# qiaozhijian/VCR-Net

Measured on AMD Instinct MI355X. Metric: point-cloud pairs/sec (N=1024, batch 16 per GPU), higher is better.
Workload: dtype f32; 1 GPU; BASELINE configs[1]: ModelNet40-like whole-to-whole registration, N=1024, batch=16 pairs per GPU, LPDNet(k=20)+Transformer+VcpTopK+SVD, iter=1, fp32; synthetic object clouds with the reference's transform recipe; LPD-pretrained emb_nn + seeded Transformer weights; num_points=1024, batch_per_gpu=16, global_batch=16, k=20, iters=1, parallelism=dp1 (pairs sharded per rank), entry_point=vcrnet_amd.module.vcrnetIter(net, src, tgt, iter) -> vcr_vcrnet_iter_f32

## Files before the change

vcr-net_amd/csrc/forward.hip:

```cpp
#include "common.h"

namespace {

enum Launch : int {
  STEM, KNN, TIE_REPLAY, EDGECONV, SN1_PQ, GATHERMAX, CONV3,
  ENCDEC_QKV, ENCDEC_SELF, WO_PAIR, FFN1_CROSS_Q, MERGED_ENC_FFN2,
  ENC_QKV = ENCDEC_QKV, ENC_SELF, ENC_WO, ENC_FFN1, ENC_FFN2, DEC_QKV, DEC_SELF, DEC_SELF_WO, DEC_CROSS_Q,
  DEC_CROSS_KV, CROSS_ATT, DEC_CROSS_WO, DEC_FFN1, DEC_FFN2, DEC_NORM, HEAD, HEAD2,
  END = HEAD2
};
static_assert(MERGED_ENC_FFN2 < DEC_CROSS_KV, "the merged first sublayers end in front of the positions both forms share");

struct Plan {
  struct Req { void** slot; size_t bytes; int birth, death; size_t off; };
  static constexpr int MAXR = 96;
  Req r[MAXR];
  int n = 0;
  bool overflow = false;
  bool flat = false;
  template <class T> void want(T*& field, size_t count, int birth, int death) {
    field = nullptr;
    if (count == 0) return;
    if (flat) { birth = 0; death = 1 << 30; }
    if (n >= MAXR) { overflow = true; return; }
    r[n++] = Req{reinterpret_cast<void**>(&field), (count * sizeof(T) + 255) & ~(size_t)255, birth, death, 0};
  }
  size_t solve(unsigned char* base) {
    int order[MAXR];
    for (int i = 0; i < n; ++i) order[i] = i;
    for (int i = 1; i < n; ++i) {
      const int x = order[i];
      int j = i - 1;
      while (j >= 0 && r[order[j]].bytes < r[x].bytes) { order[j + 1] = order[j]; --j; }
      order[j + 1] = x;
    }
    size_t total = 0;
    for (int oi = 0; oi < n; ++oi) {
      Req& q = r[order[oi]];
      size_t off = 0;
      for (bool moved = true; moved;) {
        moved = false;
        for (int pj = 0; pj < oi; ++pj) {
          const Req& p = r[order[pj]];
          if (p.death < q.birth || q.death < p.birth) continue;
          if (off < p.off + p.bytes && p.off < off + q.bytes) { off = p.off + p.bytes; moved = true; }
        }
      }
      q.off = off;
      if (off + q.bytes > total) total = off + q.bytes;
    }
    for (int i = 0; i < n; ++i) *r[i].slot = base + r[i].off;
    return total;
  }
};

struct Ws {
  float *xyz4, *feat64, *sq64, *pq1, *cat, *pq3, *emb;
  int32_t *idx1, *idx3, *ties;
  unsigned char* tie_work[2]; size_t tie_work_each;
  float* feat64t;
  float *feat_p, *xyz4_p, *cen64, *cen4, *sq_p, *c64_sq, *c64_rad, *c64_max, *c4_rad, *c4_max;
  int32_t *perm, *ord_ok;
  float *qkv, *att, *attx, *e1, *e2, *hid, *d1, *d2, *d3, *qc, *kvc, *embf, *side4, *csplit, *asplit;
  float* corr_ba;
  long asplit_floats;
  float *st_emb, *st_e1, *st_e2, *st_d1, *st_d2;
  float *rowstat, *keymass; uint8_t* keep;
  float* xsplit;
  float* xscore;
  int32_t* xorder;
  float *rstat, *cstat, *colsum, *rowsum, *score;
  float* rsplit;
  int32_t *sel_s, *sel_t, *amax, *pick;
  float *so_e, *to_e, *so_s, *to_s, *peak;
  float *eh1, *eh2, *eh3;
  float *cur_cf, *Ri, *ti, *Rb, *tb;
  size_t bytes;
};
inline size_t tgt_cache_floats(int B, int N, int E) { return (size_t)2 * B * N * 5 * E; }

inline int overlap_k1(int N, double o2) { return (int)((double)N * 0.84 * o2); }
inline int overlap_k2(int N, double o2) { return (int)((double)overlap_k1(N, o2) * 0.52 * o2); }

constexpr int KNN_ORDERED_MIN_N = 2048;
inline int merged_encdec(const vcr_vcrnet_weights* W) {
  return W->has_pointer == 1 && (W->linear_mode == 0 || W->split.encdec_qkv) && W->fold_encdec_qkv.w && W->fold_encdec_qkv.colsum &&
         W->fold_encdec_qkv.bias;
}

extern "C" int vcr_linear_shapes_(const vcr_linear_args* a, const vcr_linear_args* b, int* shape_a, int* shape_b);
extern "C" int vcr_knn_forms_(const vcr_knn_args* a, const vcr_knn_args* b, int* ordered, int* inline_a, int* inline_b);
extern "C" int vcr_sdpa_forms_(const vcr_sdpa_args* a, int* nsplit, int* persistent);
extern "C" long vcr_sdpa_split_floats_(size_t rows, int heads, int ldo, long nbatch, int nq, int cus);

Ws carve(void* base, const vcr_vcrnet_weights* W, int B, int N, int cus, int pass = 0) {
  const int k = W->k, E = W->E, F = W->F, heads = W->heads;
  const bool merged = merged_encdec(W) != 0;
  Plan pl;
  pl.flat = W->workspace_flat != 0;
  const size_t M = (size_t)2 * B * N;
  Ws w{};
  pl.want(w.xyz4, M * 4, STEM, END);   pl.want(w.feat64, M * 64, STEM, EDGECONV);   pl.want(w.sq64, M, STEM, TIE_REPLAY);
  pl.want(w.idx1, M * k, KNN, EDGECONV);   pl.want(w.idx3, M * k, KNN, GATHERMAX);   pl.want(w.ties, 2 * (1 + M), STEM, TIE_REPLAY);
  {
    const size_t slots = vcr_knn_tie_slot_bytes(2 * B, N);
    w.tie_work_each = (k > 20 && slots <= ((size_t)1 << 30)) ? slots : vcr_knn_tie_work_bytes(N);
    w.tie_work_each = (w.tie_work_each + 255) & ~(size_t)255;
  }
  pl.want(w.tie_work[0], w.tie_work_each ? 2 * w.tie_work_each : 0, KNN, TIE_REPLAY);
  pl.want(w.pq1, M * 256, STEM, SN1_PQ);   pl.want(w.cat, M * 512, EDGECONV, CONV3);   pl.want(w.pq3, M * 512, SN1_PQ, GATHERMAX);
  pl.want(w.emb, M * E, STEM, DEC_NORM);
  pl.want(w.qkv, M * 3 * E * (merged ? 2 : 1), merged ? ENCDEC_QKV : ENC_QKV, merged ? ENCDEC_SELF : DEC_SELF);
  pl.want(w.att, M * E * (merged ? 2 : 1), merged ? ENCDEC_SELF : ENC_SELF, merged ? WO_PAIR : DEC_SELF_WO);
  pl.want(w.e1, M * E, merged ? WO_PAIR : ENC_WO, merged ? MERGED_ENC_FFN2 : ENC_FFN2);
  pl.want(w.e2, M * E, merged ? MERGED_ENC_FFN2 : ENC_FFN2, DEC_CROSS_KV);
  pl.want(w.hid, M * F, merged ? FFN1_CROSS_Q : ENC_FFN1, DEC_FFN2);
  pl.want(w.d1, M * E, merged ? WO_PAIR : DEC_SELF_WO, DEC_CROSS_WO);
  pl.want(w.qc, M * E, merged ? FFN1_CROSS_Q : DEC_CROSS_Q, CROSS_ATT);   pl.want(w.kvc, M * 2 * E, DEC_CROSS_KV, CROSS_ATT);
  pl.want(w.attx, M * E, CROSS_ATT, DEC_CROSS_WO);
  pl.want(w.d2, M * E, DEC_CROSS_WO, END);
  pl.want(w.d3, M * E, DEC_FFN2, END);
  pl.want(w.embf, M * E, DEC_NORM, END);  pl.want(w.side4, M * 4, DEC_NORM, END);
  pl.want(w.csplit, VCR_PAIRSCORE_MAX_SPLIT * (M / 2) * 8, HEAD, END);
  pl.want(w.corr_ba, (size_t)B * N * 4, HEAD2, END);
  w.asplit_floats = vcr_sdpa_split_floats_(2 * M, heads, E, 2L * B, N, cus);
  pl.want(w.asplit, (size_t)w.asplit_floats, merged ? ENCDEC_SELF : ENC_SELF, CROSS_ATT);
  const size_t sn = M * (E / 64) * 2;
  pl.want(w.st_emb, sn, CONV3, DEC_QKV);
  pl.want(w.st_e1, sn, merged ? WO_PAIR : ENC_WO, merged ? FFN1_CROSS_Q : ENC_FFN1);
  pl.want(w.st_e2, sn, merged ? MERGED_ENC_FFN2 : ENC_FFN2, DEC_CROSS_KV);
  pl.want(w.st_d1, sn, merged ? WO_PAIR : DEC_SELF_WO, merged ? FFN1_CROSS_Q : DEC_CROSS_Q);
  pl.want(w.st_d2, sn, DEC_CROSS_WO, DEC_FFN1);
  const size_t K1 = (size_t)overlap_k1(N, W->overlap2), K2 = (size_t)overlap_k2(N, W->overlap2), B1 = (size_t)B;
  if (W->partial) {
    pl.want(w.rowstat, M * heads * 2, CROSS_ATT, CROSS_ATT); pl.want(w.keymass, M, CROSS_ATT, CROSS_ATT); pl.want(w.keep, M, CROSS_ATT, CROSS_ATT);
    pl.want(w.xsplit, VCR_SDPA_MAX_SPLIT * M * heads * 2, CROSS_ATT, CROSS_ATT);
    const size_t xs = M * heads * ((N + 31) & ~31);
    const int xmb = W->xscore_limit_mb;
    const size_t xlimit = xmb > 0 ? (size_t)xmb << 20 : xmb < 0 ? 0 : (size_t)4 << 30;
    pl.want(w.xscore, xs * 4 <= xlimit ? xs : 0, CROSS_ATT, CROSS_ATT);
    pl.want(w.xorder, M, CROSS_ATT, CROSS_ATT);
    pl.want(w.rstat, B1 * N * 2, HEAD, END); pl.want(w.cstat, B1 * N * 2, HEAD, END);
    pl.want(w.rsplit, VCR_PAIRSCORE_MAX_SPLIT * B1 * N * 2, HEAD, END);
    pl.want(w.rowsum, 2 * B1 * N, HEAD, END);
    pl.want(w.score, B1 * N * ((N + 31) & ~31), HEAD, END);
    pl.want(w.sel_s, 2 * B1 * K1, HEAD, END);
    pl.want(w.amax, B1 * K1, HEAD, END);     pl.want(w.pick, B1 * (K2 ? K2 : 1), HEAD, END);
    pl.want(w.so_e, 2 * B1 * K1 * E, HEAD, END);
    pl.want(w.so_s, 2 * B1 * K1 * 4, HEAD, END);
    pl.want(w.peak, B1 * K1 * 2, HEAD, END);
  }
  if (W->emb_kind == 1 && k != 20 && k != 40) {
    const size_t Mk = M * k;
    pl.want(w.eh1, Mk * 64, EDGECONV, GATHERMAX); pl.want(w.eh2, Mk * 64, EDGECONV, GATHERMAX);
    pl.want(w.eh3, Mk * 128, EDGECONV, GATHERMAX);
  }
  pl.want(w.cur_cf, (size_t)B * 3 * N, STEM, END);
  pl.want(w.Ri, (size_t)B * 9, STEM, END); pl.want(w.ti, (size_t)B * 3, STEM, END);
  pl.want(w.Rb, (size_t)B * 9, STEM, END); pl.want(w.tb, (size_t)B * 3, STEM, END);
  w.bytes = pl.solve(reinterpret_cast<unsigned char*>(base)) + 256;
  bool bad = pl.overflow;
  w.tie_work[1] = w.tie_work[0] ? w.tie_work[0] + w.tie_work_each : nullptr;
  if (W->partial) {
    w.colsum = w.rowsum + B1 * N;
    w.sel_t = w.sel_s + B1 * K1;
    w.to_e = w.so_e + B1 * K1 * E;
    w.to_s = w.so_s + B1 * K1 * 4;
  }
  if (pass != 0) {
    float* c = reinterpret_cast<float*>(static_cast<unsigned char*>(base) + w.bytes);
    w.emb = c;   c += M * E;
    w.d1 = c;    c += M * E;
    w.qc = c;    c += M * E;
    w.kvc = c;
  }
  w.feat64t = E >= 64 ? w.emb : nullptr;
  {
    const size_t T = (size_t)2 * B * ((N + 15) / 16);
    float* p = w.emb + M * 64;
    auto take = [&p](size_t n) { float* q = p; p += n; return q; };
    w.feat_p = take(M * 64);  w.xyz4_p = take(M * 4);  w.cen64 = take(T * 64);  w.cen4 = take(T * 4);  w.sq_p = take(M);
    w.perm = reinterpret_cast<int32_t*>(take(M));
    w.c64_sq = take(T);  w.c64_rad = take(T);  w.c64_max = take(T);  w.c4_rad = take(T);  w.c4_max = take(T);
    w.ord_ok = reinterpret_cast<int32_t*>(take(2 * B));
    if (pass != 0 && p > w.emb + B1 * N * E) bad = true;
  }
  if (bad) w.bytes = ~(size_t)0;
  return w;
}

__global__ __launch_bounds__(256) void zero_i32_kernel(int32_t* p, long n) {
  const long i = (long)blockIdx.x * 256 + threadIdx.x;
  if (i < n) p[i] = 0;
}

struct Runner {
  hipStream_t stream; vcr_trace* tr; int rc = 0;
  int shape_rows = 0;
  int plan_nbatch = 0;
  bool sdpa_split = false;
  float* pv_split = nullptr; long pv_split_floats = 0;
  int linear_variant = 0;
  int sdpa_variant = 0;
  vcr_knn_args deferred[2];
  int n_deferred = 0;

  void pin_shape(vcr_linear_args& a, vcr_linear_args* b = nullptr, int full_rows = 0) {
    const int fm = full_rows ? full_rows : shape_rows;
    if (!shape_rows || a.M >= fm || (a.variant & (16 | 1024))) return;
    vcr_linear_args fa = a, fb = b ? *b : a;
    fa.M = fm; fb.M = fm;
    int sa = 0, sb = 0;
    if (vcr_linear_shapes_(&fa, b ? &fb : nullptr, &sa, &sb) != VCR_OK) return;
    a.variant |= sa ? 16 : 1024;
    if (b) b->variant |= sb ? 16 : 1024;
  }
  bool ok(int r) { if (rc == 0 && r != 0) rc = r; return rc == 0; }
  template <class F> bool run(const char* name, F&& launch) {
    if (rc) return false;
    if (tr) {
      if (tr->count < VCR_TRACE_MAX) tr->names[tr->count] = name;
      if (tr->events && tr->count < tr->capacity) (void)hipEventRecord((hipEvent_t)tr->events[tr->count], stream);
      ++tr->count;
    }
    return ok(launch());
  }
  void finish() {
    if (tr && tr->events && tr->count < tr->capacity) (void)hipEventRecord((hipEvent_t)tr->events[tr->count], stream);
  }

  vcr_linear_args linear_args(const float* x, int ldx, const float* w, const float* b, float* y, int ldy, int M, int N, int K,
                              int relu, const float* res = nullptr, int ldr = 0, const float* ln_stats = nullptr,
                              const float* ln_colsum = nullptr, float* stats_out = nullptr) {
    vcr_linear_args a{x, ldx, w, b, res, ldr, y, ldy, M, N, K, relu};
    if (ln_stats) { a.ln_stats_in = ln_stats; a.ln_nseg = K / 64; a.ln_colsum = ln_colsum; a.ln_eps = 1e-6f; }
    a.stats_out = stats_out;
    a.variant = linear_variant;
    return a;
  }
  struct Lin { const char* name; vcr_linear_args a; const void* split; };
  bool linear(const Lin& l) {
    return run(l.name, [&] {
      vcr_linear_args a = l.a;
      if (!l.split) pin_shape(a);
      return l.split ? vcr_linear_bf16x3_f32(&a, l.split, stream) : vcr_linear_f32(&a, stream);
    });
  }
  bool linear(const char* nm, const float* x, int ldx, const float* w, const void* wsplit, const float* b, float* y,
              int ldy, int M, int N, int K, int relu, const float* res = nullptr, int ldr = 0,
              const float* ln_stats = nullptr, const float* ln_colsum = nullptr, float* stats_out = nullptr) {
    return linear({nm, linear_args(x, ldx, w, b, y, ldy, M, N, K, relu, res, ldr, ln_stats, ln_colsum, stats_out), wsplit});
  }
  bool linear2(const char* nm, vcr_linear_args a, vcr_linear_args b) {
    return run(nm, [&] {
      pin_shape(a, &b);
      return vcr_linear_pair_f32(&a, &b, stream);
    });
  }
  bool norm(const char* nm, const float* x, const vcr_norm_w& n, float* y, int M, int E,
            const float* res = nullptr, const float* xyz4 = nullptr, float* side4 = nullptr) {
    return run(nm, [&] {
      vcr_layernorm_args a{x, E, n.ln_a, n.ln_b, 1e-6f, res, E, y, E, M, E, xyz4, side4};
      return vcr_layernorm_f32(&a, stream);
    });
  }
  bool sdpa(const char* nm, const float* q, int ldq, const float* k, int ldk, const float* v, int ldv, float* out,
            int ldo, int nb, int heads, int nq, int nk, int shift, const uint8_t* keep = nullptr,
            float* rowstat = nullptr, float* score_out = nullptr, int ld_score = 0, int ngroups = 1, long in_group_stride = 0,
            long out_group_stride = 0, float* split_work = nullptr, long split_floats = 0) {
    return run(nm, [&] {
      vcr_sdpa_args a{q, ldq, k, ldk, v, ldv, out, ldo, nb, heads, nq, nk, 1.0f / sqrtf(128.f), shift, keep, rowstat,
                      score_out, ld_score};
      a.split_work = split_work ? split_work : out ? pv_split : nullptr;
      a.split_work_floats = split_work ? split_floats : out ? pv_split_floats : 0;
      if (ngroups > 1) {
        a.ngroups = ngroups; a.q_group_stride = a.k_group_stride = a.v_group_stride = in_group_stride;
        a.out_group_stride = out_group_stride;
      }
      a.variant = sdpa_variant;
      if (plan_nbatch > nb) a.plan_nbatch = plan_nbatch;
      return (sdpa_split && out && !rowstat && !score_out) ? vcr_sdpa_bf16x3_f32(&a, stream) : vcr_sdpa_f32(&a, stream);
    });
  }
  bool pairscore(const char* nm, const vcr_pairscore_args& a) {
    return run(nm, [&] { return vcr_pairscore_f32(&a, stream); });
  }
  bool rank(const char* nm, const float* values, int stride, int nb, int n, int K, int32_t* order, uint8_t* mask,
            int largest) {
    return run(nm, [&] {
      vcr_rankselect_args a{values, nb, n, K, order, mask, largest, stride};
      return vcr_rankselect_f32(&a, stream);
    });
  }
  bool gather(const char* nm, const float* in, int ld, int n_in, const int32_t* idx, int nb, int n_out, int C,
              float* out, const int32_t* via = nullptr, int n_via = 0) {
    return run(nm, [&] {
      vcr_gather_args a{in, ld, n_in, idx, nb, n_out, C, out, C, via, n_via};
      return vcr_gather_rows_f32(&a, stream);
    });
  }

  void knn(const char* nm, vcr_knn_args a) {
    a.tie_zeroed = 1;
    run(nm, [&] { return vcr_knn_f32(&a, stream); });
  }
  void knn_pair(const char* nm, vcr_knn_args a64, vcr_knn_args a3) {
    run(nm, [&] {
      a64.tie_zeroed = a3.tie_zeroed = 1;
      a64.tie_defer = a3.tie_defer = 1;
      n_deferred = 0;
      int inl64 = 0, inl3 = 0;
      (void)vcr_knn_forms_(&a64, &a3, nullptr, &inl64, &inl3);
      if (!inl64) deferred[n_deferred++] = a64;
      if (!inl3) deferred[n_deferred++] = a3;
      return vcr_knn_pair_f32(&a64, &a3, stream);
    });
  }
  void knn_ties() {
    if (n_deferred) run("knn:ties", [&] { return vcr_knn_ties_f32(&deferred[0], n_deferred == 2 ? &deferred[1] : nullptr, stream); });
    n_deferred = 0;
  }
  void copy_idx(const char* nm, int32_t* dst, const int32_t* src, size_t n) {
    run(nm, [&] { return vcr_copy_d2d(dst, src, n * sizeof(int32_t), stream); });
  }

  void cross_attention(const vcr_vcrnet_weights* W, const vcr_vcrnet_io* io, const Ws& w, int B, int N) {
    const int E = W->E, H = W->heads, nb = 2 * B, dk = E / H;
    const uint8_t* keep = nullptr;
    if (W->partial) {
      const int nkeep = (int)((double)N * W->overlap2);
      if (io->force_keys) {
        if (sdpa_split && W->F < 2 * E) { ok(VCR_EUNSUPPORTED); return; }
        copy_idx("select:dec.cross.keys.forced", w.xorder, io->force_keys, (size_t)nb * nkeep);
      } else if (w.xscore) {
        const int ldS = (N + 31) & ~31;
        sdpa("sdpa:dec.cross.stats", w.qc, E, w.kvc, 2 * E, nullptr, 0, nullptr, 0, nb, H, N, N, B, nullptr, w.rowstat,
             w.xscore, ldS, 1, 0, 0, w.xsplit, (long)VCR_SDPA_MAX_SPLIT * nb * H * N * 2);
        run("scoremass:dec.cross.keymass", [&] {
          vcr_keymass_args a{w.xscore, ldS, nb, H, N, N, w.rowstat, B, w.keymass};
          return vcr_keymass_f32(&a, stream);
        });
      } else {
        sdpa("sdpa:dec.cross.stats", w.qc, E, w.kvc, 2 * E, nullptr, 0, nullptr, 0, nb, H, N, N, B, nullptr, w.rowstat, nullptr, 0,
             1, 0, 0, w.xsplit, (long)VCR_SDPA_MAX_SPLIT * nb * H * N * 2);
        for (int h = 0; h < H; ++h) {
          vcr_pairscore_args a{};
          a.own = w.kvc + h * dk; a.ld_own = 2 * E; a.str = w.qc + h * dk; a.ld_str = E;
          a.nbatch = nb; a.n_own = N; a.n_str = N; a.E = dk; a.score = 1; a.scale = 1.0f / sqrtf((float)dk);
          a.str_batch_shift = B; a.op = 2; a.str_stat2 = w.rowstat + (size_t)h * N * 2;
          a.str_stat_batch_stride = (long)H * N * 2; a.mass = w.keymass; a.accumulate = h > 0;
          pairscore("pairscore:dec.cross.keymass", a);
        }
      }
      if (!io->force_keys) rank("select:dec.cross.keys", w.keymass, 1, nb, N, nkeep, w.xorder, w.keep, 1);
      if (io->out_keys) copy_idx("select:dec.cross.keys.out", io->out_keys, w.xorder, (size_t)nb * nkeep);
      vcr_sdpa_args xa{w.qc, E, w.kvc, 2 * E, w.kvc + E, 2 * E, w.attx, E, nb, H, N, nkeep, 1.0f / sqrtf(128.f), B};
      xa.key_index = w.xorder; xa.nk_src = N;
      if (!sdpa_split && vcr_sdpa_forms_(&xa, nullptr, nullptr) == VCR_OK) {
        run("sdpa:dec.cross", [&] { return vcr_sdpa_f32(&xa, stream); });
        return;
      }
      if (W->F >= 2 * E) {
        gather("select:gather.kv", w.kvc, 2 * E, N, w.xorder, nb, nkeep, 2 * E, w.hid);
        sdpa("sdpa:dec.cross", w.qc, E, w.hid, 2 * E, w.hid + E, 2 * E, w.attx, E, nb, H, N, nkeep, B);
        return;
      }
      keep = w.keep;
    }
    sdpa("sdpa:dec.cross", w.qc, E, w.kvc, 2 * E, w.kvc + E, 2 * E, w.attx, E, nb, H, N, N, B, keep);
  }

  void partial_head(const vcr_vcrnet_weights* W, const vcr_vcrnet_io* io, const Ws& w, int B, int N) {
    const int E = W->E, M1 = B * N;
    const int K1 = overlap_k1(N, W->overlap2), K2 = overlap_k2(N, W->overlap2);
    const float *se = w.embf, *te = w.embf + (size_t)M1 * E, *ss = w.side4, *ts = w.side4 + (size_t)M1 * 4;
    auto stats = [&](const char* nm, const float* own, const float* str, const float* os, const float* sd, int no,
                     int ns, float* stat2, int32_t* amax, float* score_out, int ld_score) {
      vcr_pairscore_args a{};
      a.own = own; a.ld_own = E; a.str = str; a.ld_str = E; a.own_side4 = os; a.str_side4 = sd;
      a.nbatch = B; a.n_own = no; a.n_str = ns; a.E = E; a.score = 0; a.scale = 1.f; a.op = 1;
      a.stat2 = stat2; a.argmax = amax; a.score_out = score_out; a.ld_score = ld_score;
      a.split_work = amax ? nullptr : w.rsplit;
      a.split_work_floats = amax ? 0 : (long)VCR_PAIRSCORE_MAX_SPLIT * B * N * 2;
      pairscore(nm, a);
    };
    const int ldS = (N + 31) & ~31;
    const bool forced_sets = io->force_sel_src && io->force_sel_tgt;
    if (!forced_sets) {
      stats("pairscore:head.scores", se, te, ss, ts, N, N, w.rstat, nullptr, w.score, ldS);
      run("scoremass:head", [&] {
        vcr_scoremass_args a{w.score, ldS, B, N, N, w.rstat, w.cstat, w.colsum, w.rowsum};
        return vcr_scoremass_f32(&a, stream);
      });
    }
    if (forced_sets) {
      copy_idx("select:head.tgt.forced", w.sel_t, io->force_sel_tgt, (size_t)B * K1);
      copy_idx("select:head.src.forced", w.sel_s, io->force_sel_src, (size_t)B * K1);
    } else {
      rank("select:head.src+tgt", w.rowsum, 1, 2 * B, N, K1, w.sel_s, nullptr, 1);
    }
    if (io->out_sel_tgt) copy_idx("select:head.tgt.out", io->out_sel_tgt, w.sel_t, (size_t)B * K1);
    if (io->out_sel_src) copy_idx("select:head.src.out", io->out_sel_src, w.sel_s, (size_t)B * K1);
    gather("select:gather.emb", se, E, N, w.sel_s, 2 * B, K1, E, w.so_e);
    gather("select:gather.xyz", ss, 4, N, w.sel_s, 2 * B, K1, 4, w.so_s);
    if (!(io->force_argmax && io->force_pairs))
      stats("pairscore:head.copair", w.so_e, w.to_e, w.so_s, w.to_s, K1, K1, w.peak, w.amax, nullptr, 0);
    if (io->force_argmax) copy_idx("select:head.argmax.forced", w.amax, io->force_argmax, (size_t)B * K1);
    if (io->force_pairs) copy_idx("select:head.pairs.forced", w.pick, io->force_pairs, (size_t)B * K2);
    else rank("select:head.pairs", w.peak + 1, 2, B, K1, K2, w.pick, nullptr, 0);
    if (io->out_argmax) copy_idx("select:head.argmax.out", io->out_argmax, w.amax, (size_t)B * K1);
    if (io->out_pairs) copy_idx("select:head.pairs.out", io->out_pairs, w.pick, (size_t)B * K2);
    gather("select:gather.srcK", w.so_s, 4, K1, w.pick, B, K2, 4, io->src4);
    gather("select:gather.corrK", w.to_s, 4, K1, w.pick, B, K2, 4, io->corr4, w.amax, K1);
    run("rigid_svd:ab", [&] {
      vcr_rigid_svd_args a{io->src4, 4, io->corr4, 4, B, K2, io->R_ab, io->t_ab, io->R_ba, io->t_ba, nullptr};
      return vcr_rigid_svd_f32(&a, stream);
    });
  }
};

int forward_impl(const vcr_vcrnet_weights* W, const vcr_vcrnet_io* io, void* workspace, size_t ws_bytes,
                 vcr_stream_t stream, vcr_trace* tr, bool last = true, int pass = 0) {
  if (!W || !io || !workspace || !io->src_cf || !io->tgt_cf || !io->corr4 || !io->src4 || !io->R_ab || !io->t_ab)
    return VCR_EINVAL;
  const int B = io->B, N = io->N, E = W->E, F = W->F, k = W->k;
  if (B <= 0 || N <= 0 || E != 512 || W->heads * 128 != E || k <= 0 || k + 1 > N) return VCR_EINVAL;
  if (k > 62 || N > 65535) return VCR_EUNSUPPORTED;
  if (W->emb_kind < 0 || W->emb_kind > 2) return VCR_EINVAL;
  if (W->emb_kind == 2 && !(W->c1_w && W->c1_b && W->c2_w && W->c2_b && W->pointnet.c3_w && W->pointnet.c3_b && W->pointnet.c4_w &&
                            W->pointnet.c4_b && W->pointnet.c5_w && W->pointnet.c5_b))
    return VCR_EINVAL;
  if (W->has_pointer == 1 && (F % 128)) return VCR_EINVAL;
  if (W->has_pointer == 1 &&
      !(W->fold_enc_qkv.w && W->fold_enc_ffn1.w && W->fold_dec_qkv.w && W->fold_dec_cross_q.w &&
        W->fold_dec_cross_kv.w && W->fold_dec_ffn1.w))
    return VCR_EINVAL;
  if (((uintptr_t)workspace) & 255) return VCR_EINVAL;
  if (W->head_mode < 0 || W->head_mode > 2 || W->linear_mode < 0 || W->linear_mode > 2) return VCR_EINVAL;
  for (int ms : {W->linear_mfma, W->linear_bk})
    if (ms != 0 && ms != 16 && ms != 32) return VCR_EINVAL;
  if ((W->linear_bm != 0 && W->linear_bm != 96 && W->linear_bm != 128) || (W->linear_bm == 96 && W->linear_mfma == 32)) return VCR_EINVAL;
  if (W->knn_waves != 0 && W->knn_waves != 1 && W->knn_waves != 8) return VCR_EINVAL;
  if (W->partial) {
    if (W->has_pointer != 1 || (W->cycle && W->head_mode == 0)) return VCR_EUNSUPPORTED;
    if (!(W->overlap2 > 0.0 && W->overlap2 <= 1.0) || (int)((double)N * W->overlap2) < 1) return VCR_EINVAL;
    if (W->head_mode == 0 && overlap_k2(N, W->overlap2) < 3) return VCR_EINVAL;
  }
  if (!W->partial && (io->force_keys || io->force_sel_src || io->force_sel_tgt || io->force_argmax || io->force_pairs))
    return VCR_EINVAL;
  if ((io->force_sel_src != nullptr) != (io->force_sel_tgt != nullptr)) return VCR_EINVAL;
  Ws w = carve(workspace, W, B, N, vcr_cu_count(), pass);
  if (ws_bytes < w.bytes) return VCR_EWORKSPACE;
  if (pass != 0 && ws_bytes < w.bytes + tgt_cache_floats(B, N, E) * sizeof(float)) return VCR_EINVAL;
  const int M1 = B * N, M2 = 2 * M1;
  const bool half = pass == 2;
  const int Bq = half ? B : 2 * B, Mq = half ? M1 : M2;
#define NM(site) (half ? site "@src" : site)
  Runner R{(hipStream_t)stream, tr};
  R.shape_rows = half ? M2 : 0;
  R.plan_nbatch = half ? 2 * B : 0;
  hipLaunchKernelGGL(zero_i32_kernel, dim3((unsigned)((M2 + 2 + 255) / 256)), dim3(256), 0, R.stream, w.ties, (long)(M2 + 2));
  R.ok(VCR_LAUNCH_RC());
#define SP(site) (W->linear_mode != 0 ? W->split.site : nullptr)
  R.sdpa_split = W->linear_mode == 2;
  R.sdpa_variant = W->sdpa_variant;
  R.pv_split = w.asplit; R.pv_split_floats = w.asplit_floats;
  R.linear_variant = (W->linear_mfma == 16 ? 16 : W->linear_mfma == 32 ? 1024 : 0) | (W->linear_bk == 16 ? 64 : W->linear_bk == 32 ? 8 : 0) |
                     (W->linear_bm == 96 ? 2048 : W->linear_bm == 128 ? 4096 : 0);

  const float* stats_for_ln = W->has_pointer == 1 ? w.st_emb : nullptr;
  if (W->emb_kind == 1) {
    for (int c = 0; c < (half ? 1 : 2); ++c) {
      R.run(c ? "pointwise:tgt" : "pointwise:src", [&] {
        return vcr_rows4_pq_f32(c ? io->tgt_cf : io->src_cf, w.xyz4 + (size_t)c * M1 * 4, B, N, W->dgcnn.c1_wpq, 32,
                                W->dgcnn.c1_bpq, 128, w.pq1 + (size_t)c * M1 * 128, 128, R.stream);
      });
    }
    {
      vcr_knn_args a3{(uint32_t)sizeof(vcr_knn_args), w.xyz4, 4, nullptr, Bq, N, 4, k, w.idx3, w.ties + 1 + M2, M2};
      a3.tie_work = w.tie_work[0]; a3.tie_work_bytes = w.tie_work_each;
      R.knn(NM("knn:xyz"), a3);
    }
    const int Mk = Mq * k;
    auto conv_max = [&](const char* nm, const float* x, int K, const float* wt, const float* bias, float* y, int Nout,
                        int col) {
      R.run(nm, [&] {
        vcr_linear_args a{x, K, wt, bias, nullptr, 0, y, Nout, Mk, Nout, K, 1};
        a.segmax_out = w.cat + col; a.ld_segmax = 512; a.seg_k = k;
        a.variant = R.linear_variant;
        R.pin_shape(a, nullptr, M2 * k);
        return vcr_linear_f32(&a, R.stream);
      });
    };
    if (k == 20 || k == 40) {
      R.run(NM("edgeconv:dg_chain"), [&] {
        vcr_edgechain_args a{w.pq1, 128, w.idx3, k, Mq, N, W->dgcnn.c2_w, W->dgcnn.c2_b, W->dgcnn.c3_w, W->dgcnn.c3_b,
                             W->dgcnn.c4_w, W->dgcnn.c4_b, w.cat, 512};
        return vcr_edgechain_f32(&a, R.stream);
      });
    } else {
      R.run(NM("gathermax:dg_c1"), [&] {
        vcr_edgerows_args a{w.pq1, 128, 64, w.idx3, k, Mq, N, w.eh1, 64, w.cat, 512, 512};
        return vcr_edgerows_f32(&a, R.stream);
      });
      conv_max(NM("linear:dg_c2"), w.eh1, 64, W->dgcnn.c2_w, W->dgcnn.c2_b, w.eh2, 64, 64);
      conv_max(NM("linear:dg_c3"), w.eh2, 64, W->dgcnn.c3_w, W->dgcnn.c3_b, w.eh3, 128, 128);
      conv_max(NM("linear:dg_c4"), w.eh3, 128, W->dgcnn.c4_w, W->dgcnn.c4_b, nullptr, 256, 256);
    }
    R.linear(NM("linear:conv3"), w.cat, 512, W->dgcnn.c5_w, nullptr, W->dgcnn.c5_b, w.emb, E, Mq, E, 512, 1, nullptr, 0, nullptr,
             nullptr, const_cast<float*>(stats_for_ln));
  } else if (W->emb_kind == 2) {
    R.run(NM("pointwise:src+tgt"), [&] {
      vcr_pointwise_args a{io->src_cf, B, N, W->c1_w, W->c1_b, W->c2_w, W->c2_b, w.xyz4, w.feat64, w.sq64, half ? nullptr : io->tgt_cf,
                           half ? 0 : B};
      return vcr_pointwise_f32(&a, R.stream);
    });
    R.linear(NM("linear:pn_c3"), w.feat64, 64, W->pointnet.c3_w, nullptr, W->pointnet.c3_b, w.pq1, 64, Mq, 64, 64, 1);
    R.linear(NM("linear:pn_c4"), w.pq1, 64, W->pointnet.c4_w, nullptr, W->pointnet.c4_b, w.cat, 128, Mq, 128, 64, 1);
    R.linear(NM("linear:pn_c5"), w.cat, 128, W->pointnet.c5_w, nullptr, W->pointnet.c5_b, w.emb, E, Mq, E, 128, 1, nullptr, 0, nullptr,
             nullptr, const_cast<float*>(stats_for_ln));
  } else {
  const bool pq_fused = W->linear_mode == 0;
  R.run(pq_fused ? NM("pointwise:src+tgt+dg1_pq") : NM("pointwise:src+tgt"), [&] {
    vcr_pointwise_args a{io->src_cf, B, N, W->c1_w, W->c1_b, W->c2_w, W->c2_b, w.xyz4, w.feat64, w.sq64, half ? nullptr : io->tgt_cf,
                         half ? 0 : B};
    if (pq_fused) { a.pq_w = W->dg1_wpq; a.pq_b = W->dg1_bpq; a.pq = w.pq1; a.ldpq = 256; }
    a.feat64t = w.feat64t;
    return vcr_pointwise_f32(&a, R.stream);
  });
  const int32_t* rank_perm = nullptr;
  {
    vcr_knn_args a64{(uint32_t)sizeof(vcr_knn_args), w.feat64, 64, w.sq64, Bq, N, 64, k, w.idx1, w.ties, M2, W->knn_waves};
    vcr_knn_args a3{(uint32_t)sizeof(vcr_knn_args), w.xyz4, 4, nullptr, Bq, N, 4, k, w.idx3, w.ties + 1 + M2, M2};
    a64.tie_work = w.tie_work[0]; a3.tie_work = w.tie_work[1];
    a64.tie_work_bytes = a3.tie_work_bytes = w.tie_work_each;
    a64.xt = w.feat64t;
    int pair_ordered = 0;
    if (R.rc == 0 && W->E >= 256 && N >= KNN_ORDERED_MIN_N && N <= 8192 && (k == 20 || k == 40) && W->knn_waves == 0 &&
        vcr_knn_forms_(&a64, &a3, &pair_ordered, nullptr, nullptr) == VCR_OK && pair_ordered) {
      R.run(NM("knn:rank"), [&] {
        vcr_knn_order_args o{w.xyz4, w.feat64t, 64, w.sq64, Bq, N, w.perm, w.xyz4_p, w.cen4, w.c4_rad, w.c4_max, w.feat_p, w.sq_p,
                             w.cen64, w.c64_sq, w.c64_rad, w.c64_max, w.ord_ok, nullptr, 0.f};
        return vcr_knn_order_f32(&o, R.stream);
      });
      a64.perm = a3.perm = w.perm;
      a64.ord_ok = w.ord_ok;
      rank_perm = w.perm;
      a64.xp = w.feat_p; a64.sqp = w.sq_p; a64.cen = w.cen64; a64.cen_sq = w.c64_sq; a64.cen_rad = w.c64_rad; a64.cen_sqmax = w.c64_max;
      a3.xp = w.xyz4_p; a3.cen = w.cen4; a3.cen_rad = w.c4_rad; a3.cen_sqmax = w.c4_max;
    }
    R.knn_pair(NM("knn:feat64+xyz"), a64, a3);
  }
  if (!pq_fused) R.linear(NM("linear:dg1_pq"), w.feat64, 64, W->dg1_wpq, SP(dg1_pq), W->dg1_bpq, w.pq1, 256, Mq, 256, 64, 0);
  R.knn_ties();
  R.run(NM("edgeconv:dg1_dg2"), [&] {
    vcr_edgeconv_args a{w.pq1, 256, w.idx1, k, Mq, N, W->dg2_w, W->dg2_b, w.cat, 512, w.cat + 128, 512};
    return W->linear_mode != 0 && (k == 20 || k == 40) ? vcr_edgeconv_bf16x3_f32(&a, R.stream) : vcr_edgeconv_f32(&a, R.stream);
  });
  R.linear(NM("linear:sn1_pq"), w.cat + 128, 512, W->sn1_wpq, SP(sn1_pq), W->sn1_bpq, w.pq3, 512, Mq, 512, 128, 0);
  R.run(NM("gathermax:sn1"), [&] {
    vcr_gathermax_args a{w.pq3, 512, 256, w.idx3, k, Mq, N, w.cat + 256, 512};
    a.order = rank_perm;
    return vcr_gathermax_f32(&a, R.stream);
  });
  R.linear(NM("linear:conv3"), w.cat, 512, W->c3_w, SP(c3), W->c3_b, w.emb, E, Mq, E, 512, 1, nullptr, 0, nullptr, nullptr,
           W->has_pointer == 1 ? w.st_emb : nullptr);

  }
  if (W->has_pointer != 1) { R.shape_rows = 0; R.plan_nbatch = 0; }

  const float* head_emb = w.embf;
  if (W->has_pointer == 1) {
    const int H = W->heads;
    const bool merged = merged_encdec(W) != 0;
    const float* att_dec = merged ? w.att + (size_t)M2 * E : w.att;
    using Lin = Runner::Lin;
    const Lin enc_wo{NM("linear:enc.wo"), R.linear_args(w.att, E, W->enc_self.wo, W->enc_self.bo, w.e1, E, Mq, E, E, 0, w.emb, E,
                                                         nullptr, nullptr, w.st_e1), SP(enc_wo)};
    const Lin dec_self_wo{NM("linear:dec.self.wo"), R.linear_args(att_dec, E, W->dec_self.wo, W->dec_self.bo, w.d1, E, Mq, E, E, 0,
                                                                  w.emb, E, nullptr, nullptr, w.st_d1), SP(dec_self_wo)};
    const Lin enc_ffn1{NM("linear:enc.ffn1"), R.linear_args(w.e1, E, W->fold_enc_ffn1.w, W->fold_enc_ffn1.bias, w.hid, F, Mq, F, E, 1,
                                                            nullptr, 0, w.st_e1, W->fold_enc_ffn1.colsum), SP(enc_ffn1)};
    const Lin dec_cross_q{NM("linear:dec.cross.q"), R.linear_args(w.d1, E, W->fold_dec_cross_q.w, W->fold_dec_cross_q.bias, w.qc, E, Mq,
                                                                  E, E, 0, nullptr, 0, w.st_d1, W->fold_dec_cross_q.colsum),
                          SP(dec_cross_q)};
    const Lin enc_ffn2{NM("linear:enc.ffn2"), R.linear_args(w.hid, F, W->enc_ffn.w2, W->enc_ffn.b2, w.e2, E, Mq, E, F, 0, w.e1, E,
                                                            nullptr, nullptr, w.st_e2), SP(enc_ffn2)};
    if (merged) {
      R.linear(NM("linear:encdec.qkv"), w.emb, E, W->fold_encdec_qkv.w, SP(encdec_qkv), W->fold_encdec_qkv.bias, w.qkv, 6 * E, Mq, 6 * E, E, 0,
               nullptr, 0, w.st_emb, W->fold_encdec_qkv.colsum);
      R.sdpa(NM("sdpa:encdec.self"), w.qkv, 6 * E, w.qkv + E, 6 * E, w.qkv + 2 * E, 6 * E, w.att, E, Bq, H, N, N, 0, nullptr, nullptr,
             nullptr, 0, 2, 3 * E, (long)M2 * E);
      if (W->linear_mode != 0) {
        R.linear(enc_wo); R.linear(dec_self_wo); R.linear(enc_ffn1); R.linear(dec_cross_q); R.linear(enc_ffn2);
      } else {
        R.linear2(NM("linear:enc.wo+dec.self.wo"), enc_wo.a, dec_self_wo.a);
        R.linear2(NM("linear:enc.ffn1+dec.cross.q"), enc_ffn1.a, dec_cross_q.a);
        R.linear(enc_ffn2);
      }
    } else {
      R.linear(NM("linear:enc.qkv"), w.emb, E, W->fold_enc_qkv.w, SP(enc_qkv), W->fold_enc_qkv.bias, w.qkv, 3 * E, Mq, 3 * E, E, 0,
               nullptr, 0, w.st_emb, W->fold_enc_qkv.colsum);
      R.sdpa(NM("sdpa:enc.self"), w.qkv, 3 * E, w.qkv + E, 3 * E, w.qkv + 2 * E, 3 * E, w.att, E, Bq, H, N, N, 0);
      R.linear(enc_wo); R.linear(enc_ffn1); R.linear(enc_ffn2);
      R.linear(NM("linear:dec.qkv"), w.emb, E, W->fold_dec_qkv.w, SP(dec_qkv), W->fold_dec_qkv.bias, w.qkv, 3 * E, Mq, 3 * E, E, 0,
               nullptr, 0, w.st_emb, W->fold_dec_qkv.colsum);
      R.sdpa(NM("sdpa:dec.self"), w.qkv, 3 * E, w.qkv + E, 3 * E, w.qkv + 2 * E, 3 * E, w.att, E, Bq, H, N, N, 0);
      R.linear(dec_self_wo); R.linear(dec_cross_q);
    }
    R.linear(NM("linear:dec.cross.kv"), w.e2, E, W->fold_dec_cross_kv.w, SP(dec_cross_kv), W->fold_dec_cross_kv.bias, w.kvc, 2 * E, Mq, 2 * E, E, 0,
             nullptr, 0, w.st_e2, W->fold_dec_cross_kv.colsum);
    R.shape_rows = 0; R.plan_nbatch = 0;
    R.cross_attention(W, io, w, B, N);
    R.linear("linear:dec.cross.wo", w.attx, E, W->dec_cross.wo, SP(dec_cross_wo), W->dec_cross.bo, w.d2, E, M2, E, E, 0, w.d1, E,
             nullptr, nullptr, w.st_d2);
    R.linear("linear:dec.ffn1", w.d2, E, W->fold_dec_ffn1.w, SP(dec_ffn1), W->fold_dec_ffn1.bias, w.hid, F, M2, F, E, 1, nullptr, 0,
             w.st_d2, W->fold_dec_ffn1.colsum);
    R.linear("linear:dec.ffn2", w.hid, F, W->dec_ffn.w2, SP(dec_ffn2), W->dec_ffn.b2, w.d3, E, M2, E, F, 0, w.d2, E);
    R.norm("layernorm:dec.norm+res", w.d3, W->dec_norm, w.embf, M2, E, w.emb, w.xyz4, w.side4);
  } else {
    R.run("layernorm:rowside", [&] {
      vcr_rowside_args a{w.emb, E, M2, E, W->has_pointer == 2 ? 2.f : 1.f, w.embf, E, w.xyz4, w.side4};
      return vcr_rowside_f32(&a, R.stream);
    });
  }

  const bool hard_pairs = W->partial && W->head_mode == 0;
  const float* side = w.side4;
  if (W->head_mode == 2) {
    if (!W->att_w0 || !W->att_w1) return VCR_EINVAL;
    R.linear("linear:head.att.src", w.embf, E, W->att_w0, nullptr, W->att_b0, w.d3, E, M1, E, E, 0);
    R.linear("linear:head.att.tgt", w.embf + (size_t)M1 * E, E, W->att_w1, nullptr, W->att_b1, w.d3 + (size_t)M1 * E, E,
             M1, E, E, 0);
    R.run("layernorm:rowside.att", [&] {
      vcr_rowside_args a{w.d3, E, M2, E, 1.f, nullptr, E, w.xyz4, w.side4};
      return vcr_rowside_f32(&a, R.stream);
    });
    head_emb = w.d3;
  }
  auto soft_head = [&](const char* nm, size_t q0, size_t k0, float* corr) {
    R.run(nm, [&] {
      vcr_softcorr_args a{head_emb + q0 * E, E, head_emb + k0 * E, E, side + q0 * 4, side + k0 * 4,
                          corr, B, N, N, E, W->head_mode == 1 ? 1 : 0, 1.0f / sqrtf((float)E), w.csplit,
                          (long)VCR_PAIRSCORE_MAX_SPLIT * B * N * 8};
      return vcr_softcorr_f32(&a, R.stream);
    });
  };
  if (hard_pairs) {
    R.partial_head(W, io, w, B, N);
  } else {
    soft_head("softcorr:head", 0, (size_t)M1, io->corr4);
    R.run("rigid_svd:ab", [&] {
      const int c = vcr_copy_d2d(io->src4, w.xyz4, (size_t)M1 * 4 * sizeof(float), R.stream);
      vcr_rigid_svd_args a{w.xyz4, 4, io->corr4, 4, B, N, io->R_ab, io->t_ab, io->R_ba, io->t_ba, nullptr};
      const int s = vcr_rigid_svd_f32(&a, R.stream);
      return c ? c : s;
    });
    if (W->cycle) {
      if (!io->R_ba || !io->t_ba) return VCR_EINVAL;
      if (W->head_mode == 2) {
        R.linear("linear:head.att.ba.src", w.embf, E, W->att_w1, nullptr, W->att_b1, w.d2, E, M1, E, E, 0);
        R.linear("linear:head.att.ba.tgt", w.embf + (size_t)M1 * E, E, W->att_w0, nullptr, W->att_b0, w.d2 + (size_t)M1 * E,
                 E, M1, E, E, 0);
        R.run("layernorm:rowside.att.ba", [&] {
          vcr_rowside_args a{w.d2, E, M2, E, 1.f, nullptr, E, w.xyz4, w.side4};
          return vcr_rowside_f32(&a, R.stream);
        });
        head_emb = w.d2;
      }
      soft_head("softcorr:head.ba", (size_t)M1, 0, w.corr_ba);
      R.run("rigid_svd:ba", [&] {
        vcr_rigid_svd_args a{w.xyz4 + (size_t)M1 * 4, 4, w.corr_ba, 4, B, N, io->R_ba, io->t_ba, nullptr, nullptr, nullptr};
        return vcr_rigid_svd_f32(&a, R.stream);
      });
    }
  }
  if (R.rc == 0 && io->emb_out) R.ok(vcr_copy_d2d(io->emb_out, w.embf, (size_t)M2 * E * sizeof(float), R.stream));
  if (last) R.finish();
#undef SP
#undef NM
  return R.rc;
}

__global__ __launch_bounds__(256) void pose_step_kernel(const float* __restrict__ Ri, const float* __restrict__ ti,
                                                        const float* in_cf, float* out_cf, int N, int compose,
                                                        float* Rf, float* tf, float* Rba, float* tba) {
  const int b = blockIdx.y;
  float r[9], t[3];
  for (int i = 0; i < 9; ++i) r[i] = Ri[b * 9 + i];
  for (int i = 0; i < 3; ++i) t[i] = ti[b * 3 + i];
  if (out_cf) {
    const int n = blockIdx.x * 256 + threadIdx.x;
    if (n < N) {
      const float* p = in_cf + (size_t)b * 3 * N + n;
      const float x = p[0], y = p[N], z = p[2 * (size_t)N];
      float* o = out_cf + (size_t)b * 3 * N + n;
      for (int c = 0; c < 3; ++c) o[(size_t)c * N] = fmaf(r[c * 3 + 2], z, fmaf(r[c * 3 + 1], y, r[c * 3] * x)) + t[c];
    }
  }
  if (compose == 2 && blockIdx.x == 0 && threadIdx.x == 0) {
    for (int i = 0; i < 3; ++i) {
      for (int j = 0; j < 3; ++j) Rba[b * 9 + i * 3 + j] = r[j * 3 + i];
      tba[b * 3 + i] = -fmaf(r[6 + i], t[2], fmaf(r[3 + i], t[1], r[i] * t[0]));
    }
  } else if (compose && blockIdx.x == 0 && threadIdx.x == 0) {
    float f[9], g[3], nf[9], ng[3];
    for (int i = 0; i < 9; ++i) f[i] = Rf[b * 9 + i];
    for (int i = 0; i < 3; ++i) g[i] = tf[b * 3 + i];
    for (int i = 0; i < 3; ++i) {
      for (int j = 0; j < 3; ++j) nf[i * 3 + j] = fmaf(r[i * 3 + 2], f[6 + j], fmaf(r[i * 3 + 1], f[3 + j], r[i * 3] * f[j]));
      ng[i] = fmaf(r[i * 3 + 2], g[2], fmaf(r[i * 3 + 1], g[1], r[i * 3] * g[0])) + t[i];
    }
    for (int i = 0; i < 9; ++i) Rf[b * 9 + i] = nf[i];
    for (int i = 0; i < 3; ++i) tf[b * 3 + i] = ng[i];
    for (int i = 0; i < 3; ++i) {
      for (int j = 0; j < 3; ++j) Rba[b * 9 + i * 3 + j] = nf[j * 3 + i];
      tba[b * 3 + i] = -fmaf(nf[6 + i], ng[2], fmaf(nf[3 + i], ng[1], nf[i] * ng[0]));
    }
  }
}

}

static int weights_take(const vcr_vcrnet_weights* user, vcr_vcrnet_weights* mine) {
  return vcr_take_args(user, mine, offsetof(vcr_vcrnet_weights, fold_encdec_qkv));
}

extern "C" size_t vcr_vcrnet_workspace_bytes(const vcr_vcrnet_weights* UW, int B, int N) {
  vcr_vcrnet_weights Wn;
  const vcr_vcrnet_weights* W = &Wn;
  if (weights_take(UW, &Wn) || B <= 0 || N <= 0) return 0;
  return carve(nullptr, W, B, N, vcr_cu_count()).bytes;
}

static bool iter_reuse_applies(const vcr_vcrnet_weights* W, int iters) { return iters > 1 && W->iter_reuse != 1; }
extern "C" size_t vcr_vcrnet_iter_workspace_bytes(const vcr_vcrnet_weights* UW, int B, int N, int iters) {
  vcr_vcrnet_weights Wn;
  const vcr_vcrnet_weights* W = &Wn;
  if (weights_take(UW, &Wn) || B <= 0 || N <= 0 || iters < 1) return 0;
  const size_t base = carve(nullptr, W, B, N, vcr_cu_count()).bytes;
  return base + (iter_reuse_applies(W, iters) ? tgt_cache_floats(B, N, W->E) * sizeof(float) : 0);
}

extern "C" int vcr_vcrnet_pairs(const vcr_vcrnet_weights* UW, int N) {
  vcr_vcrnet_weights Wn;
  const vcr_vcrnet_weights* W = &Wn;
  if (weights_take(UW, &Wn) || N <= 0) return 0;
  return (W->partial && W->head_mode == 0) ? overlap_k2(N, W->overlap2) : N;
}

extern "C" int vcr_vcrnet_forward_f32(const vcr_vcrnet_weights* UW, const vcr_vcrnet_io* io, void* ws, size_t bytes,
                                      vcr_stream_t stream) {
  vcr_vcrnet_weights Wn;
  if (weights_take(UW, &Wn)) return VCR_EINVAL;
  return forward_impl(&Wn, io, ws, bytes, stream, nullptr);
}

extern "C" int vcr_vcrnet_forward_traced_f32(const vcr_vcrnet_weights* UW, const vcr_vcrnet_io* io, void* ws,
                                             size_t bytes, vcr_stream_t stream, vcr_trace* tr) {
  vcr_vcrnet_weights Wn;
  if (weights_take(UW, &Wn)) return VCR_EINVAL;
  if (tr) tr->count = 0;
  return forward_impl(&Wn, io, ws, bytes, stream, tr);
}

extern "C" int vcr_vcrnet_iter_f32(const vcr_vcrnet_weights* UW, const vcr_vcrnet_io* io, int iters, void* ws,
                                   size_t bytes, vcr_stream_t stream, vcr_trace* tr) {
  vcr_vcrnet_weights Wn;
  const vcr_vcrnet_weights* W = &Wn;
  if (weights_take(UW, &Wn)) return VCR_EINVAL;
  if (!W || !io || iters < 1 || !io->R_ba || !io->t_ba) return VCR_EINVAL;
  if (tr) tr->count = 0;
  const int B = io->B, N = io->N;
  if (B <= 0 || N <= 0) return VCR_EINVAL;
  if (iters == 1) {
    const int rc = forward_impl(W, io, ws, bytes, stream, tr, !W->cycle);
    if (rc || !W->cycle) return rc;
    Runner R{(hipStream_t)stream, tr};
    R.run("pose:inverse", [&] {
      hipLaunchKernelGGL(pose_step_kernel, dim3(1, B), dim3(64), 0, R.stream, io->R_ab, io->t_ab, nullptr, nullptr, N, 2, nullptr,
                         nullptr, io->R_ba, io->t_ba);
      return VCR_LAUNCH_RC();
    });
    R.finish();
    return R.rc;
  }
  const Ws w = carve(ws, W, B, N, vcr_cu_count());
  if (bytes < w.bytes) return VCR_EWORKSPACE;
  const bool reuse = iter_reuse_applies(W, iters) && bytes >= w.bytes + tgt_cache_floats(B, N, W->E) * sizeof(float);
  const size_t nkeys = W->partial ? (size_t)2 * B * (int)((double)N * W->overlap2) : 0;
  const size_t nsel = W->partial ? (size_t)B * overlap_k1(N, W->overlap2) : 0;
  const size_t npair = W->partial ? (size_t)B * overlap_k2(N, W->overlap2) : 0;
  for (int it = 0; it < iters; ++it) {
    vcr_vcrnet_io step = *io;
    if (it > 0) { step.src_cf = w.cur_cf; step.R_ab = w.Ri; step.t_ab = w.ti; step.R_ba = w.Rb; step.t_ba = w.tb; }
    if (it + 1 < iters) step.emb_out = nullptr;
    auto at = [it](auto* p, size_t n) { return p ? p + (size_t)it * n : p; };
    step.force_keys = at(io->force_keys, nkeys);       step.out_keys = at(io->out_keys, nkeys);
    step.force_sel_src = at(io->force_sel_src, nsel);  step.out_sel_src = at(io->out_sel_src, nsel);
    step.force_sel_tgt = at(io->force_sel_tgt, nsel);  step.out_sel_tgt = at(io->out_sel_tgt, nsel);
    step.force_argmax = at(io->force_argmax, nsel);    step.out_argmax = at(io->out_argmax, nsel);
    step.force_pairs = at(io->force_pairs, npair);     step.out_pairs = at(io->out_pairs, npair);
    const bool last = it + 1 == iters;
    const int rc = forward_impl(W, &step, ws, bytes, stream, tr, false, reuse ? (it == 0 ? 1 : 2) : 0);
    if (rc) return rc;
    if (last && it == 0) break;
    Runner R{(hipStream_t)stream, tr};
    R.run("pose:step", [&] {
      hipLaunchKernelGGL(pose_step_kernel, dim3((N + 255) / 256, B), dim3(256), 0, R.stream, step.R_ab, step.t_ab, step.src_cf,
                         last ? nullptr : w.cur_cf, N, it > 0 ? 1 : 0, io->R_ab, io->t_ab, io->R_ba, io->t_ba);
      return VCR_LAUNCH_RC();
    });
    if (R.rc) return R.rc;
    if (last) R.finish();
  }
  return VCR_OK;
}

extern "C" int vcr_pose_step_f32(const vcr_pose_step_args* a, vcr_stream_t stream) {
  if (!a || !a->R_i || !a->t_i || a->B <= 0 || a->compose < 0 || a->compose > 2) return VCR_EINVAL;
  if ((a->out_cf != nullptr) != (a->in_cf != nullptr) || (a->out_cf && a->N <= 0)) return VCR_EINVAL;
  if (a->compose && (!a->R_ba || !a->t_ba)) return VCR_EINVAL;
  if (a->compose == 1 && (!a->R_f || !a->t_f)) return VCR_EINVAL;
  if (!a->compose && !a->out_cf) return VCR_OK;
  const int gx = a->out_cf ? (a->N + 255) / 256 : 1;
  hipLaunchKernelGGL(pose_step_kernel, dim3(gx, a->B), dim3(a->out_cf ? 256 : 64), 0, (hipStream_t)stream, a->R_i, a->t_i,
                     a->in_cf, a->out_cf, a->N, a->compose, a->R_f, a->t_f, a->R_ba, a->t_ba);
  return VCR_LAUNCH_RC();
}

extern "C" const char* vcr_strerror(int code) {
  switch (code) {
    case VCR_OK: return "ok";
    case VCR_EINVAL: return "invalid argument (shape, pitch, alignment or null pointer)";
    case VCR_EWORKSPACE: return "workspace too small";
    case VCR_EUNSUPPORTED: return "unsupported configuration";
    default: return code > 0 ? hipGetErrorString((hipError_t)code) : "unknown error";
  }
}

extern "C" int vcr_abi_version(void) { return VCR_ABI_VERSION; }

extern "C" int vcr_event_create(void** ev) {
  if (!ev) return VCR_EINVAL;
  hipEvent_t e;
  const hipError_t rc = hipEventCreate(&e);
  *ev = rc == hipSuccess ? (void*)e : nullptr;
  return (int)rc;
}
extern "C" int vcr_event_destroy(void* ev) { return ev ? (int)hipEventDestroy((hipEvent_t)ev) : VCR_EINVAL; }
extern "C" int vcr_event_record(void* ev, vcr_stream_t stream) {
  return ev ? (int)hipEventRecord((hipEvent_t)ev, (hipStream_t)stream) : VCR_EINVAL;
}
extern "C" int vcr_event_elapsed_ms(void* start, void* stop, float* ms) {
  if (!start || !stop || !ms) return VCR_EINVAL;
  return (int)hipEventElapsedTime(ms, (hipEvent_t)start, (hipEvent_t)stop);
}
```

vcr-net_amd/csrc/pairscore.hip:

```cpp
#include "common.h"

namespace {

constexpr float LOG2E = 1.4426950408889634f;

__device__ __forceinline__ bool argmax_before(float v, int i, float bv, int bi) {
  const bool vn = v != v, bn = bv != bv;
  return vn ? (!bn || i < bi) : (!bn && (v > bv || (v == bv && i < bi)));
}

template <int OP, int OT>
__global__ __launch_bounds__(128 * OT * 2, (OT == 1 ? 2 : 1)) void pairscore_kernel(vcr_pairscore_args p, int nsplit) {
  extern __shared__ __attribute__((aligned(16))) unsigned char smem[];
  constexpr int NW = 4 * OT;
  constexpr int NO = 32 * OT;
  const int QP = p.E + 4;
  float* Os = reinterpret_cast<float*>(smem);
  float* mg = Os + NO * QP;
  const int t = threadIdx.x, lane = t & 63, w = t >> 6;
  const int half = lane >> 5, l31 = lane & 31;
  int bx, b;
  xcd_chunk2(bx, b);
  const int sp = bx % nsplit;
  bx /= nsplit;
  const int o0 = bx * NO;
  const int sb = (b + p.str_batch_shift) % p.nbatch;
  const int chunks = p.E / 64;

  {
    const int per_row = p.E / 4;
    for (int i = t; i < NO * per_row; i += 64 * NW) {
      const int row = i / per_row, c4 = (i % per_row) * 4;
      const int orow = min(o0 + row, p.n_own - 1);
      st4(&Os[row * QP + c4], ld4(p.own + ((size_t)b * p.n_own + orow) * p.ld_own + c4));
    }
  }
  size_t own_row[OT];
  float own_norm[OT];
#pragma unroll
  for (int ot = 0; ot < OT; ++ot) {
    own_row[ot] = (size_t)b * p.n_own + min(o0 + 32 * ot + l31, p.n_own - 1);
    own_norm[ot] = p.score == 1 ? 0.f : p.own_side4[own_row[ot] * 4 + 3];
  }
  __syncthreads();

  const int ntiles_all = (p.n_str + 31) / 32;
  const int per_split = (ntiles_all + nsplit - 1) / nsplit, t0 = sp * per_split;
  const int ntiles = max(0, min(ntiles_all, t0 + per_split) - t0);
  const int my_tiles = max(0, (ntiles - w + NW - 1) / NW);
  const int nflat = my_tiles * chunks;
  const float* sbase = p.str + (size_t)sb * p.n_str * p.ld_str;
  const float* sside = p.str_side4 ? p.str_side4 + (size_t)sb * p.n_str * 4 : nullptr;
  const float* sstat = (OP == 2) ? p.str_stat2 + (size_t)sb * p.str_stat_batch_stride : nullptr;

  f32x4 bufA[8], bufB[8];
  auto load_chunk = [&](int flat, f32x4* dst) {
    const int tile = t0 + w + NW * (flat / chunks), c = flat % chunks;
    const int row = min(tile * 32 + l31, p.n_str - 1);
    const float* kp = sbase + (size_t)row * p.ld_str + 64 * c + 4 * half;
#pragma unroll
    for (int g = 0; g < 8; ++g) dst[g] = ld4(kp + 8 * g);
  };

  float m[OT], l[OT], ox[OT], oy[OT], oz[OT];
  float best[OT]; int bidx[OT];
  float mass[OT];
  f32x16 s[OT];
#pragma unroll
  for (int ot = 0; ot < OT; ++ot) {
    m[ot] = VCR_NEG_INF; l[ot] = ox[ot] = oy[ot] = oz[ot] = 0.f; best[ot] = VCR_NEG_INF; bidx[ot] = 0x7fffffff;
    mass[ot] = 0.f; s[ot] = f32x16{0};
  }
  f32x16 tot[OT];
  auto compute = [&](int flat, const f32x4* kf) {
    const int tile = t0 + w + NW * (flat / chunks), c = flat % chunks;
#pragma unroll
    for (int ot = 0; ot < OT; ++ot) s[ot] = f32x16{0};
#pragma unroll
    for (int g = 0; g < 8; ++g) {
#pragma unroll
      for (int ot = 0; ot < OT; ++ot) {
        const f32x4 qv = ld4(&Os[(32 * ot + l31) * QP + 64 * c + 8 * g + 4 * half]);
#pragma unroll
        for (int e = 0; e < 4; ++e) s[ot] = mfma32(kf[g][e], qv[e], s[ot]);
      }
    }
#pragma unroll
    for (int ot = 0; ot < OT; ++ot) {
      if (c == 0) tot[ot] = s[ot];
      else tot[ot] += s[ot];
    }
    if (c != chunks - 1) return;
    float rn = 0.f;
    if (p.score == 2) rn = sside[(size_t)min(tile * 32 + l31, p.n_str - 1) * 4 + 3];
    f32x4 side[16];
    if (OP == 0 || p.score == 0) {
#pragma unroll
      for (int r = 0; r < 16; ++r) side[r] = ld4(sside + (size_t)min(tile * 32 + acc_row(r, half), p.n_str - 1) * 4);
    }
#pragma unroll
    for (int ot = 0; ot < OT; ++ot) {
      f32x16& sc16 = tot[ot];
      if (p.score == 0) sc16 = mfma32(half == 0 ? 1.f : 0.f, half == 0 ? -0.5f * own_norm[ot] : 0.f, sc16);
      else if (p.score == 2) sc16 = mfma32(half == 0 ? -0.5f * rn : 0.f, half == 0 ? 1.f : 0.f, sc16);
      float mt = VCR_NEG_INF;
#pragma unroll
      for (int r = 0; r < 16; ++r) {
        const int j = tile * 32 + acc_row(r, half);
        float sc;
        if (p.score == 0) sc = 2.f * sc16[r] - side[r][3];
        else if (p.score == 2) sc = 2.f * sc16[r] - own_norm[ot];
        else sc = sc16[r] * p.scale;
        sc16[r] = j < p.n_str ? sc : VCR_NEG_INF;
        mt = fmaxf(mt, sc16[r]);
      }
      if (OP == 1 && p.score_out && o0 + 32 * ot + l31 < p.n_own) {
        float* srow = p.score_out + (own_row[ot] * (size_t)p.ld_score) + tile * 32 + 4 * half;
#pragma unroll
        for (int r4 = 0; r4 < 4; ++r4)
          st4(srow + 8 * r4, f32x4{sc16[4 * r4], sc16[4 * r4 + 1], sc16[4 * r4 + 2], sc16[4 * r4 + 3]});
      }
      if (OP == 2) {
#pragma unroll
        for (int r = 0; r < 16; ++r) {
          const int jc = min(tile * 32 + acc_row(r, half), p.n_str - 1);
          const float ms = sstat[(size_t)jc * 2], ls = sstat[(size_t)jc * 2 + 1];
          mass[ot] += __builtin_amdgcn_exp2f((sc16[r] - ms) * LOG2E) / ls;
        }
        continue;
      }
      if (OP == 1) {
#pragma unroll
        for (int r = 0; r < 16; ++r) {
          const int j = tile * 32 + acc_row(r, half);
          if (sc16[r] > best[ot] || (sc16[r] != sc16[r] && best[ot] == best[ot])) { best[ot] = sc16[r]; bidx[ot] = j; }
        }
      }
      mt = fmaxf(mt, xhalf(mt));
      const float m_new = fmaxf(m[ot], mt);
      const float alpha = __builtin_amdgcn_exp2f((m[ot] - m_new) * LOG2E);
      float ls = 0.f, ax = 0.f, ay = 0.f, az = 0.f;
#pragma unroll
      for (int r = 0; r < 16; ++r) {
        const float pr = __builtin_amdgcn_exp2f((sc16[r] - m_new) * LOG2E);
        ls += pr;
        if (OP == 0) { ax = fmaf(pr, side[r][0], ax); ay = fmaf(pr, side[r][1], ay); az = fmaf(pr, side[r][2], az); }
      }
      l[ot] = l[ot] * alpha + ls;
      if (OP == 0) { ox[ot] = ox[ot] * alpha + ax; oy[ot] = oy[ot] * alpha + ay; oz[ot] = oz[ot] * alpha + az; }
      m[ot] = m_new;
    }
  };

  if (nflat > 0) {
    load_chunk(0, bufA);
    int f = 0;
    for (; f + 2 < nflat; f += 2) {
      load_chunk(f + 1, bufB);
      __builtin_amdgcn_sched_barrier(0);
      compute(f, bufA);
      load_chunk(f + 2, bufA);
      __builtin_amdgcn_sched_barrier(0);
      compute(f + 1, bufB);
    }
    load_chunk(f + 1, bufB);
    __builtin_amdgcn_sched_barrier(0);
    compute(f, bufA);
    compute(f + 1, bufB);
  }

#pragma unroll
  for (int ot = 0; ot < OT; ++ot) {
    float* g = mg + (w * NO + 32 * ot + l31) * 5;
    if (OP == 2) {
      mass[ot] += xhalf(mass[ot]);
      if (half == 0) g[0] = mass[ot];
    } else {
      l[ot] += xhalf(l[ot]);
      if (OP == 0) { ox[ot] += xhalf(ox[ot]); oy[ot] += xhalf(oy[ot]); oz[ot] += xhalf(oz[ot]); }
      if (OP == 1) {
        const float ob = xhalf(best[ot]);
        const int oi = __shfl_xor(bidx[ot], 32, 64);
        if (argmax_before(ob, oi, best[ot], bidx[ot])) { best[ot] = ob; bidx[ot] = oi; }
      }
      if (half == 0) {
        g[0] = m[ot]; g[1] = l[ot];
        if (OP == 0) { g[2] = ox[ot]; g[3] = oy[ot]; g[4] = oz[ot]; }
        else { g[2] = best[ot]; g[3] = __int_as_float(bidx[ot]); }
      }
    }
  }
  __syncthreads();
  if (t < NO && o0 + t < p.n_own) {
    const size_t orow = (size_t)b * p.n_own + o0 + t;
    if (OP == 2) {
      float acc = 0.f;
#pragma unroll
      for (int i = 0; i < NW; ++i) acc += mg[(i * NO + t) * 5];
      p.mass[orow] = p.accumulate ? p.mass[orow] + acc : acc;
      return;
    }
    float M = VCR_NEG_INF;
#pragma unroll
    for (int i = 0; i < NW; ++i) M = fmaxf(M, mg[(i * NO + t) * 5]);
    float L = 0.f, X = 0.f, Y = 0.f, Z = 0.f, Bv = VCR_NEG_INF;
    int Bi = 0x7fffffff;
#pragma unroll
    for (int i = 0; i < NW; ++i) {
      const float* g = mg + (i * NO + t) * 5;
      const float a = g[0] == VCR_NEG_INF ? 0.f : __builtin_amdgcn_exp2f((g[0] - M) * LOG2E);
      L = fmaf(g[1], a, L);
      if (OP == 0) { X = fmaf(g[2], a, X); Y = fmaf(g[3], a, Y); Z = fmaf(g[4], a, Z); }
      else {
        const int gi = __float_as_int(g[3]);
        if (argmax_before(g[2], gi, Bv, Bi)) { Bv = g[2]; Bi = gi; }
      }
    }
    if (OP == 0) {
      if (nsplit > 1) {
        float* pw = p.split_work + ((size_t)sp * p.nbatch * p.n_own + orow) * 8;
        st4(pw, f32x4{M, L, X, Y});
        pw[4] = Z;
      } else {
        st4(p.corr4 + orow * 4, f32x4{X / L, Y / L, Z / L, 0.f});
      }
    } else {
      float* st = nsplit > 1 ? p.split_work + (size_t)sp * p.nbatch * p.n_own * 2 : p.stat2;
      st[orow * 2] = M; st[orow * 2 + 1] = L;
      if (p.argmax) p.argmax[orow] = Bi < p.n_str ? Bi : 0;
    }
  }
}

__global__ __launch_bounds__(256) void corrmerge_kernel(const float* part, int nsplit, long rows, float* corr4) {
  const long r = (long)blockIdx.x * 256 + threadIdx.x;
  if (r >= rows) return;
  float M = VCR_NEG_INF;
  for (int s = 0; s < nsplit; ++s) M = fmaxf(M, part[((size_t)s * rows + r) * 8]);
  float L = 0.f, X = 0.f, Y = 0.f, Z = 0.f;
  for (int s = 0; s < nsplit; ++s) {
    const float* g = part + ((size_t)s * rows + r) * 8;
    const float a = g[0] == VCR_NEG_INF ? 0.f : __builtin_amdgcn_exp2f((g[0] - M) * LOG2E);
    L = fmaf(g[1], a, L); X = fmaf(g[2], a, X); Y = fmaf(g[3], a, Y); Z = fmaf(g[4], a, Z);
  }
  st4(corr4 + r * 4, f32x4{X / L, Y / L, Z / L, 0.f});
}

__global__ __launch_bounds__(256) void statmerge_kernel(const float* part, int nsplit, long rows, float* stat2) {
  const long r = (long)blockIdx.x * 256 + threadIdx.x;
  if (r >= rows) return;
  float M = VCR_NEG_INF;
  for (int s = 0; s < nsplit; ++s) M = fmaxf(M, part[((size_t)s * rows + r) * 2]);
  float L = 0.f;
  for (int s = 0; s < nsplit; ++s) {
    const float* g = part + ((size_t)s * rows + r) * 2;
    L = fmaf(g[1], g[0] == VCR_NEG_INF ? 0.f : __builtin_amdgcn_exp2f((g[0] - M) * LOG2E), L);
  }
  stat2[r * 2] = M; stat2[r * 2 + 1] = L;
}

__global__ __launch_bounds__(256) void score_colpass_kernel(vcr_scoremass_args p) {
  __shared__ float mg[4][64][3];
  const int b = blockIdx.y, lane = threadIdx.x & 63, w = threadIdx.x >> 6;
  const int j = blockIdx.x * 64 + lane, jc = min(j, p.n_cols - 1);
  const float* S = p.score + (size_t)b * p.n_rows * p.ld + jc;
  const float* rs = p.row_stat2 + (size_t)b * p.n_rows * 2;
  const int per = (p.n_rows + 3) / 4, i0 = w * per, i1 = min(p.n_rows, i0 + per);
  float cm = VCR_NEG_INF, cl = 0.f, mass = 0.f;
  auto step = [&](float v, float mi, float li) {
    mass += __builtin_amdgcn_exp2f((v - mi) * LOG2E) / li;
    if (v > cm) { cl *= __builtin_amdgcn_exp2f((cm - v) * LOG2E); cm = v; }
    cl += __builtin_amdgcn_exp2f((v - cm) * LOG2E);
  };
  int i = i0;
  for (; i + 8 <= i1; i += 8) {
    float v[8], m8[8], l8[8];
#pragma unroll
    for (int u = 0; u < 8; ++u) { v[u] = S[(size_t)(i + u) * p.ld]; m8[u] = rs[2 * (i + u)]; l8[u] = rs[2 * (i + u) + 1]; }
#pragma unroll
    for (int u = 0; u < 8; ++u) step(v[u], m8[u], l8[u]);
  }
  for (; i < i1; ++i) step(S[(size_t)i * p.ld], rs[2 * i], rs[2 * i + 1]);
  mg[w][lane][0] = cm; mg[w][lane][1] = cl; mg[w][lane][2] = mass;
  __syncthreads();
  if (w == 0 && j < p.n_cols) {
    float M = VCR_NEG_INF, L = 0.f, A = 0.f;
    for (int q = 0; q < 4; ++q) M = fmaxf(M, mg[q][lane][0]);
    for (int q = 0; q < 4; ++q) {
      L = fmaf(mg[q][lane][1], __builtin_amdgcn_exp2f((mg[q][lane][0] - M) * LOG2E), L);
      A += mg[q][lane][2];
    }
    const size_t o = (size_t)b * p.n_cols + j;
    p.col_stat2[o * 2] = M; p.col_stat2[o * 2 + 1] = L;
    p.col_mass[o] = A;
  }
}

__global__ __launch_bounds__(256) void score_rowpass_kernel(vcr_scoremass_args p) {
  const int b = blockIdx.y, lane = threadIdx.x & 63;
  const int i = blockIdx.x * 4 + (threadIdx.x >> 6);
  if (i >= p.n_rows) return;
  const float* S = p.score + ((size_t)b * p.n_rows + i) * p.ld;
  const float* cs = p.col_stat2 + (size_t)b * p.n_cols * 2;
  float acc = 0.f;
#pragma unroll 4
  for (int j = lane; j < p.n_cols; j += 64)
    acc += __builtin_amdgcn_exp2f((S[j] - cs[2 * j]) * LOG2E) / cs[2 * j + 1];
#pragma unroll
  for (int off = 32; off > 0; off >>= 1) acc += __shfl_xor(acc, off, 64);
  if (lane == 0) p.row_mass[(size_t)b * p.n_rows + i] = acc;
}

enum class PsMerge { none, corr, stat };
struct PairscorePlan {
  int op, ot;
  int nsplit;
  dim3 grid, block; int lds;
  PsMerge merge; long rows; dim3 merge_grid;
};

int pairscore_plan(const vcr_pairscore_args* a, PairscorePlan* p) {
  if (!a || !a->own || !a->str) return VCR_EINVAL;
  if (a->nbatch <= 0 || a->n_own <= 0 || a->n_str <= 0 || a->E <= 0 || (a->E % 128) || a->E > 1024) return VCR_EINVAL;
  if ((a->ld_own & 3) || (a->ld_str & 3) || a->ld_own < a->E || a->ld_str < a->E) return VCR_EINVAL;
  if (a->score < 0 || a->score > 2 || a->op < 0 || a->op > 2) return VCR_EINVAL;
  if (a->score != 1 && (!a->own_side4 || !a->str_side4)) return VCR_EINVAL;
  if (a->op == 0 && (!a->corr4 || !a->str_side4)) return VCR_EINVAL;
  if (a->op == 1 && !a->stat2) return VCR_EINVAL;
  if (a->op == 2 && (!a->mass || !a->str_stat2)) return VCR_EINVAL;
  if (a->score_out && (a->op != 1 || (a->ld_score & 3) || a->ld_score < ((a->n_str + 31) & ~31))) return VCR_EINVAL;
  const int lds2 = (64 * (a->E + 4) + 8 * 64 * 5) * 4, lds1 = (32 * (a->E + 4) + 4 * 32 * 5) * 4;
  const int ot = (lds2 <= 160 * 1024 && a->E >= 256 && !(a->variant & 1)) ? 2 : 1;
  const int lds = ot == 2 ? lds2 : lds1;
  if (lds > 160 * 1024) return VCR_EUNSUPPORTED;
  const int owner_blocks = (a->n_own + 32 * ot - 1) / (32 * ot);
  int nsplit = 1;
  if ((a->op == 0 || (a->op == 1 && !a->argmax)) && a->split_work && !(a->variant & 4)) {
    const long blocks = (long)owner_blocks * a->nbatch, slots = (long)vcr_cu_count() * (ot == 2 ? 1 : 2);
    const int ntiles = (a->n_str + 31) / 32;
    double best = (double)((blocks + slots - 1) / slots);
    const double base = best;
    for (int sp = 2; sp <= VCR_PAIRSCORE_MAX_SPLIT; ++sp) {
      if (ntiles / sp < 4 * ot || (sp - 1) * ((ntiles + sp - 1) / sp) >= ntiles) break;
      const double c = (double)((blocks * sp + slots - 1) / slots) / sp;
      const long need = (long)sp * a->nbatch * a->n_own * (a->op == 0 ? 8 : 2);
      if (need > a->split_work_floats) break;
      if (c < 0.8 * base && c < best - 1e-9) { best = c; nsplit = sp; }
    }
  }
  const long rows = (long)a->nbatch * a->n_own;
  *p = PairscorePlan{a->op, ot, nsplit, dim3(owner_blocks * nsplit, a->nbatch), dim3(256 * ot), lds,
                     nsplit == 1 ? PsMerge::none : a->op == 0 ? PsMerge::corr : PsMerge::stat, rows, dim3((unsigned)((rows + 255) / 256))};
  return VCR_OK;
}

}

extern "C" int vcr_pairscore_f32(const vcr_pairscore_args* a, vcr_stream_t stream) {
  vcr_stream_scope bound(stream);
  PairscorePlan p;
  int rc = pairscore_plan(a, &p);
  if (rc) return rc;
  hipStream_t s = (hipStream_t)stream;
#define VCR_PS(OP, OT) rc = vcr_launch<pairscore_kernel<OP, OT>>(p.grid, p.block, p.lds, s, *a, p.nsplit)
  if (p.ot == 2) { if (p.op == 0) VCR_PS(0, 2); else if (p.op == 1) VCR_PS(1, 2); else VCR_PS(2, 2); }
  else           { if (p.op == 0) VCR_PS(0, 1); else if (p.op == 1) VCR_PS(1, 1); else VCR_PS(2, 1); }
#undef VCR_PS
  if (rc || p.merge == PsMerge::none) return rc;
  if (p.merge == PsMerge::corr) hipLaunchKernelGGL(corrmerge_kernel, p.merge_grid, dim3(256), 0, s, a->split_work, p.nsplit, p.rows, a->corr4);
  else hipLaunchKernelGGL(statmerge_kernel, p.merge_grid, dim3(256), 0, s, a->split_work, p.nsplit, p.rows, a->stat2);
  return VCR_LAUNCH_RC();
}

extern "C" int vcr_scoremass_f32(const vcr_scoremass_args* a, vcr_stream_t stream) {
  if (!a || !a->score || !a->row_stat2 || !a->col_stat2 || !a->col_mass || !a->row_mass) return VCR_EINVAL;
  if (a->nbatch <= 0 || a->n_rows <= 0 || a->n_cols <= 0 || a->ld < a->n_cols) return VCR_EINVAL;
  hipStream_t s = (hipStream_t)stream;
  hipLaunchKernelGGL(score_colpass_kernel, dim3((a->n_cols + 63) / 64, a->nbatch), dim3(256), 0, s, *a);
  hipLaunchKernelGGL(score_rowpass_kernel, dim3((a->n_rows + 3) / 4, a->nbatch), dim3(256), 0, s, *a);
  return VCR_LAUNCH_RC();
}

extern "C" int vcr_softcorr_f32(const vcr_softcorr_args* a, vcr_stream_t stream) {
  if (!a || !a->qside4 || !a->kside4 || !a->corr4) return VCR_EINVAL;
  if (a->mode != 0 && a->mode != 1) return VCR_EINVAL;
  vcr_pairscore_args p{};
  p.own = a->q; p.ld_own = a->ldq; p.str = a->k; p.ld_str = a->ldk;
  p.own_side4 = a->qside4; p.str_side4 = a->kside4;
  p.nbatch = a->nbatch; p.n_own = a->nq; p.n_str = a->nk; p.E = a->E;
  p.score = a->mode; p.scale = a->scale; p.str_batch_shift = 0; p.op = 0; p.corr4 = a->corr4;
  p.split_work = a->split_work; p.split_work_floats = a->split_work_floats;
  return vcr_pairscore_f32(&p, stream);
}
```

vcr-net_amd/csrc/pointwise.hip:

```cpp
#include "common.h"

namespace {

constexpr int PTS = 64;

__global__ __launch_bounds__(256) void pointwise12_kernel(vcr_pointwise_args a) {
  __shared__ float w2t[64][64];
  __shared__ float h1s[PTS][65];
  __shared__ float w1s[64][4];
  __shared__ float b2s[64];
  const int t = threadIdx.x;
  {
    f32x4 wv[4];
#pragma unroll
    for (int u = 0; u < 4; ++u) wv[u] = ld4(a.w2 + 4 * (t + 256 * u));
#pragma unroll
    for (int u = 0; u < 4; ++u) {
      const int i = 4 * (t + 256 * u), c = i >> 6, k = i & 63;
#pragma unroll
      for (int e = 0; e < 4; ++e) w2t[k + e][c] = wv[u][e];
    }
  }
  if (t < 64) {
    w1s[t][0] = a.w1[t * 3 + 0]; w1s[t][1] = a.w1[t * 3 + 1]; w1s[t][2] = a.w1[t * 3 + 2];
    w1s[t][3] = a.b1[t]; b2s[t] = a.b2[t];
  }
  const int b = blockIdx.y;
  const int p = t >> 2, g = t & 3;
  const int n = blockIdx.x * PTS + p;
  const bool live = n < a.N;
  const int nc = live ? n : a.N - 1;
  const float* xb = b < a.B ? a.x_cf + (size_t)b * 3 * a.N : a.x_cf2 + (size_t)(b - a.B) * 3 * a.N;
  const float x = xb[nc], y = xb[a.N + nc], z = xb[2 * a.N + nc];
  __syncthreads();
#pragma unroll
  for (int j = 0; j < 16; ++j) {
    const int c = g * 16 + j;
    const float v = fmaf(w1s[c][2], z, fmaf(w1s[c][1], y, fmaf(w1s[c][0], x, w1s[c][3])));
    h1s[p][c] = fmaxf(v, 0.f);
  }
  __syncthreads();
  float acc[16];
#pragma unroll
  for (int j = 0; j < 16; ++j) acc[j] = b2s[g * 16 + j];
  for (int k = 0; k < 64; ++k) {
    const float h = h1s[p][k];
#pragma unroll
    for (int q = 0; q < 4; ++q) {
      const f32x4 w = ld4(&w2t[k][g * 16 + q * 4]);
      acc[q * 4 + 0] = fmaf(w[0], h, acc[q * 4 + 0]);
      acc[q * 4 + 1] = fmaf(w[1], h, acc[q * 4 + 1]);
      acc[q * 4 + 2] = fmaf(w[2], h, acc[q * 4 + 2]);
      acc[q * 4 + 3] = fmaf(w[3], h, acc[q * 4 + 3]);
    }
  }
  float ss = 0.f;
#pragma unroll
  for (int j = 0; j < 16; ++j) {
    acc[j] = fmaxf(acc[j], 0.f);
    ss = ss + acc[j] * acc[j];
  }
  const int base = (threadIdx.x & 63) & ~3;
  {
    const float b0 = __shfl(ss, base, 64), b1 = __shfl(ss, base + 1, 64);
    const float b2 = __shfl(ss, base + 2, 64), b3 = __shfl(ss, base + 3, 64);
    ss = ((b0 + b1) + b2) + b3;
  }
  const bool tail = live && n >= (a.N & ~31);
  if (__builtin_amdgcn_ballot_w64(tail) != 0) {
    float a4[4] = {0.f, 0.f, 0.f, 0.f};
#pragma unroll
    for (int sgrp = 0; sgrp < 4; ++sgrp) {
      if (g == sgrp) {
#pragma unroll
        for (int j = 0; j < 16; ++j) a4[j & 3] = a4[j & 3] + acc[j] * acc[j];
      }
#pragma unroll
      for (int l = 0; l < 4; ++l) a4[l] = __shfl(a4[l], base + sgrp, 64);
    }
    if (tail) ss = ((a4[0] + a4[1]) + a4[2]) + a4[3];
  }
  if (live) {
    const size_t row = (size_t)b * a.N + n;
    float* o = a.feat64 + row * 64 + g * 16;
#pragma unroll
    for (int q = 0; q < 4; ++q) st4(o + q * 4, f32x4{acc[q * 4], acc[q * 4 + 1], acc[q * 4 + 2], acc[q * 4 + 3]});
    if (a.feat64t) {
      float* ot = a.feat64t + row * 64 + g * 16;
#pragma unroll
      for (int q = 0; q < 4; ++q) st4(ot + q * 4, f32x4{acc[q], acc[4 + q], acc[8 + q], acc[12 + q]});
    }
    if (g == 0) {
      a.sq64[row] = ss;
      st4(a.xyz4 + row * 4, f32x4{x, y, z, (x * x + y * y) + z * z});
    }
  }
}

constexpr int TP = 68;
constexpr int PQW = 8;
__global__ __launch_bounds__(64 * PQW, 1) void pointwise12_pq_kernel(vcr_pointwise_args a, int tiles_per_cloud, int total_tiles) {
  extern __shared__ __attribute__((aligned(16))) float pw_smem[];
  float* wfrag = pw_smem;
  float* w1s = wfrag + 16 * 4 * 64 * 4;
  float* pqb = w1s + 64 * 4;
  float* tiles = pqb + 256;
  const int t = threadIdx.x, lane = t & 63, wave = t >> 6;
  const int q4 = lane >> 4, l15 = lane & 15;
  f32x4 w2c[4][4];
#pragma unroll
  for (int j = 0; j < 4; ++j)
#pragma unroll
    for (int g = 0; g < 4; ++g) w2c[j][g] = ld4(a.w2 + (16 * j + l15) * 64 + 16 * g + 4 * q4);
  float b2r[4];
#pragma unroll
  for (int j = 0; j < 4; ++j) b2r[j] = a.b2[16 * j + l15];
  f32x4 wq[8];
#pragma unroll
  for (int it = 0; it < 8; ++it) wq[it] = ld4(a.pq_w + 4 * (t + 64 * PQW * it));
  if (t >= 256) pqb[t - 256] = a.pq_b[t - 256];
  if (t < 64) {
    w1s[t * 4 + 0] = a.w1[t * 3 + 0]; w1s[t * 4 + 1] = a.w1[t * 3 + 1]; w1s[t * 4 + 2] = a.w1[t * 3 + 2];
    w1s[t * 4 + 3] = a.b1[t];
  }
  float w2r[4][16];
#pragma unroll
  for (int j = 0; j < 4; ++j)
#pragma unroll
    for (int g = 0; g < 4; ++g) {
      int r0 = __float_as_int(w2c[j][g][0]), r1 = __float_as_int(w2c[j][g][1]);
      int r2 = __float_as_int(w2c[j][g][2]), r3 = __float_as_int(w2c[j][g][3]);
      auto s01 = __builtin_amdgcn_permlane16_swap(r0, r1, false, false); r0 = s01[0]; r1 = s01[1];
      auto s23 = __builtin_amdgcn_permlane16_swap(r2, r3, false, false); r2 = s23[0]; r3 = s23[1];
      auto s02 = __builtin_amdgcn_permlane32_swap(r0, r2, false, false); r0 = s02[0]; r2 = s02[1];
      auto s13 = __builtin_amdgcn_permlane32_swap(r1, r3, false, false); r1 = s13[0]; r3 = s13[1];
      w2r[j][4 * g] = __int_as_float(r0); w2r[j][4 * g + 1] = __int_as_float(r1);
      w2r[j][4 * g + 2] = __int_as_float(r2); w2r[j][4 * g + 3] = __int_as_float(r3);
    }
#pragma unroll
  for (int it = 0; it < 8; ++it) {
    const int c = t + 64 * PQW * it, n = c >> 4, st = c & 15, j = n >> 4;
#pragma unroll
    for (int e = 0; e < 4; ++e) wfrag[(((j * 4 + (st >> 2)) * 64) + e * 16 + (n & 15)) * 4 + (st & 3)] = wq[it][e];
  }
  __syncthreads();
  float* T = tiles + wave * 16 * TP;
  const int p = lane >> 2, g = lane & 3;
  for (int tile = (int)blockIdx.x * PQW + wave; tile < total_tiles; tile += (int)gridDim.x * PQW) {
    const int b = tile / tiles_per_cloud, n0 = (tile - b * tiles_per_cloud) * 16;
    const float* xb = b < a.B ? a.x_cf + (size_t)b * 3 * a.N : a.x_cf2 + (size_t)(b - a.B) * 3 * a.N;
    float h[16];
    {
      const int nc = min(n0 + l15, a.N - 1);
      const float x = xb[nc], y = xb[a.N + nc], z = xb[2 * a.N + nc];
#pragma unroll
      for (int st = 0; st < 16; ++st) {
        const f32x4 w = ld4(&w1s[(4 * st + q4) * 4]);
        h[st] = fmaxf(fmaf(w[2], z, fmaf(w[1], y, fmaf(w[0], x, w[3]))), 0.f);
      }
    }
    f32x4 acc[4];
#pragma unroll
    for (int j = 0; j < 4; ++j) acc[j] = f32x4{b2r[j], b2r[j], b2r[j], b2r[j]};
#pragma unroll
    for (int st = 0; st < 16; ++st)
#pragma unroll
      for (int j = 0; j < 4; ++j) acc[j] = mfma16(h[st], w2r[j][st], acc[j]);
#pragma unroll
    for (int j = 0; j < 4; ++j)
#pragma unroll
      for (int r = 0; r < 4; ++r) T[(4 * q4 + r) * TP + 16 * j + l15] = fmaxf(acc[j][r], 0.f);
    __builtin_amdgcn_s_waitcnt(0xc07f);
    __builtin_amdgcn_wave_barrier();
    auto feature_epilogue = [&]() {
      const int n = n0 + p;
      const bool live = n < a.N;
      const int nc = live ? n : a.N - 1;
      const float x = xb[nc], y = xb[a.N + nc], z = xb[2 * a.N + nc];
      float f[16];
#pragma unroll
      for (int q = 0; q < 4; ++q) {
        const f32x4 v = ld4(&T[p * TP + 16 * g + 4 * q]);
        f[4 * q] = v[0]; f[4 * q + 1] = v[1]; f[4 * q + 2] = v[2]; f[4 * q + 3] = v[3];
      }
      float ss = 0.f;
#pragma unroll
      for (int j = 0; j < 16; ++j) ss = ss + f[j] * f[j];
      const int base = lane & ~3;
      {
        const float s0 = __shfl(ss, base, 64), s1 = __shfl(ss, base + 1, 64);
        const float s2 = __shfl(ss, base + 2, 64), s3 = __shfl(ss, base + 3, 64);
        ss = ((s0 + s1) + s2) + s3;
      }
      const bool tail = live && n >= (a.N & ~31);
      if (__builtin_amdgcn_ballot_w64(tail) != 0) {
        float a4[4] = {0.f, 0.f, 0.f, 0.f};
#pragma unroll
        for (int sgrp = 0; sgrp < 4; ++sgrp) {
          if (g == sgrp) {
#pragma unroll
            for (int j = 0; j < 16; ++j) a4[j & 3] = a4[j & 3] + f[j] * f[j];
          }
#pragma unroll
          for (int l = 0; l < 4; ++l) a4[l] = __shfl(a4[l], base + sgrp, 64);
        }
        if (tail) ss = ((a4[0] + a4[1]) + a4[2]) + a4[3];
      }
      if (live) {
        const size_t row = (size_t)b * a.N + n;
        float* o = a.feat64 + row * 64 + g * 16;
#pragma unroll
        for (int q = 0; q < 4; ++q) st4(o + q * 4, f32x4{f[q * 4], f[q * 4 + 1], f[q * 4 + 2], f[q * 4 + 3]});
        if (a.feat64t) {
          float* ot = a.feat64t + row * 64 + g * 16;
#pragma unroll
          for (int q = 0; q < 4; ++q) st4(ot + q * 4, f32x4{f[q], f[4 + q], f[8 + q], f[12 + q]});
        }
        if (g == 0) {
          a.sq64[row] = ss;
          st4(a.xyz4 + row * 4, f32x4{x, y, z, (x * x + y * y) + z * z});
        }
      }
    };
    auto pq_product = [&]() {
    float af[16];
#pragma unroll
    for (int st = 0; st < 16; ++st) af[st] = T[l15 * TP + 4 * st + q4];
#pragma unroll 1
    for (int jg = 0; jg < 4; ++jg) {
      f32x4 pa[4];
#pragma unroll
      for (int jj = 0; jj < 4; ++jj) {
        const float bq = pqb[16 * (4 * jg + jj) + l15];
        pa[jj] = f32x4{bq, bq, bq, bq};
      }
#pragma unroll
      for (int sq = 0; sq < 4; ++sq)
#pragma unroll
        for (int jj = 0; jj < 4; ++jj) {
          const f32x4 wf = ld4(&wfrag[(((4 * jg + jj) * 4 + sq) * 64 + lane) * 4]);
#pragma unroll
          for (int e = 0; e < 4; ++e) pa[jj] = mfma16(af[4 * sq + e], wf[e], pa[jj]);
        }
#pragma unroll
      for (int jj = 0; jj < 4; ++jj)
#pragma unroll
        for (int r = 0; r < 4; ++r) {
          const int n = n0 + 4 * q4 + r;
          if (n < a.N) a.pq[((size_t)b * a.N + n) * a.ldpq + 16 * (4 * jg + jj) + l15] = pa[jj][r];
        }
    }
    };
    if (wave < PQW / 2) {
      feature_epilogue();
      pq_product();
    } else {
      pq_product();
      feature_epilogue();
    }
    __builtin_amdgcn_s_waitcnt(0xc07f);
    __builtin_amdgcn_wave_barrier();
  }
}

__global__ __launch_bounds__(256) void rows4_kernel(const float* x_cf, float* xyz4, int B, int N) {
  const long i = (long)blockIdx.x * 256 + threadIdx.x;
  if (i >= (long)B * N) return;
  const int b = (int)(i / N), n = (int)(i % N);
  const float* xb = x_cf + (size_t)b * 3 * N;
  const float x = xb[n], y = xb[N + n], z = xb[2 * N + n];
  st4(xyz4 + i * 4, f32x4{x, y, z, (x * x + y * y) + z * z});
}

__global__ __launch_bounds__(256) void rows4_pq_kernel(const float* x_cf, float* xyz4, int B, int N, const float* wpq,
                                                       int ldw, const float* bpq, int C, float* pq, int ldpq) {
  const int per = C / 4, cg = threadIdx.x % per;
  const long i = (long)blockIdx.x * (256 / per) + threadIdx.x / per;
  if (i >= (long)B * N) return;
  const int b = (int)(i / N), n = (int)(i % N);
  const float* xb = x_cf + (size_t)b * 3 * N;
  const float x = xb[n], y = xb[N + n], z = xb[2 * N + n];
  if (cg == 0) st4(xyz4 + i * 4, f32x4{x, y, z, (x * x + y * y) + z * z});
  f32x4 o;
#pragma unroll
  for (int e = 0; e < 4; ++e) {
    const float* wr = wpq + (size_t)(4 * cg + e) * ldw;
    o[e] = fmaf(wr[2], z, fmaf(wr[1], y, wr[0] * x)) + bpq[4 * cg + e];
  }
  st4(pq + i * ldpq + 4 * cg, o);
}

}

extern "C" int vcr_rows4_pq_f32(const float* x_cf, float* xyz4, int B, int N, const float* wpq, int ldw, const float* bpq,
                                int C, float* pq, int ldpq, vcr_stream_t stream) {
  if (!x_cf || !xyz4 || !wpq || !bpq || !pq || B <= 0 || N <= 0) return VCR_EINVAL;
  if (C <= 0 || (C % 4) || 256 % (C / 4) || ldw < 3 || ldpq < C || (ldpq & 3) || ((uintptr_t)pq & 15)) return VCR_EINVAL;
  const int pts = 256 / (C / 4);
  hipLaunchKernelGGL(rows4_pq_kernel, dim3((unsigned)(((long)B * N + pts - 1) / pts)), dim3(256), 0, (hipStream_t)stream,
                     x_cf, xyz4, B, N, wpq, ldw, bpq, C, pq, ldpq);
  return VCR_LAUNCH_RC();
}

extern "C" int vcr_rows4_f32(const float* x_cf, float* xyz4, int B, int N, vcr_stream_t stream) {
  if (!x_cf || !xyz4 || B <= 0 || N <= 0) return VCR_EINVAL;
  hipLaunchKernelGGL(rows4_kernel, dim3((unsigned)(((long)B * N + 255) / 256)), dim3(256), 0, (hipStream_t)stream, x_cf,
                     xyz4, B, N);
  return VCR_LAUNCH_RC();
}

extern "C" int vcr_pointwise_f32(const vcr_pointwise_args* a, vcr_stream_t stream) {
  vcr_stream_scope bound(stream);
  if (!a || !a->x_cf || !a->w1 || !a->b1 || !a->w2 || !a->b2 || !a->xyz4 || !a->feat64 || !a->sq64) return VCR_EINVAL;
  if (((uintptr_t)a->w2 | (uintptr_t)a->pq_w) & 15) return VCR_EINVAL;
  if (a->B <= 0 || a->N <= 0 || a->B2 < 0 || (a->B2 > 0 && !a->x_cf2)) return VCR_EINVAL;
  if (a->pq) {
    if (!a->pq_w || !a->pq_b || a->ldpq < 256 || (a->ldpq & 3)) return VCR_EINVAL;
    const int tpc = (a->N + 15) / 16, total = tpc * (a->B + a->B2);
    const int cus = vcr_cu_count(), blocks = (total + PQW - 1) / PQW < cus ? (total + PQW - 1) / PQW : cus;
    const size_t lds = (size_t)(16 * 4 * 64 * 4 + 64 * 4 + 256 + PQW * 16 * TP) * sizeof(float);
    VCR_DYN_LDS(pointwise12_pq_kernel, lds);
    hipLaunchKernelGGL(pointwise12_pq_kernel, dim3(blocks), dim3(64 * PQW), lds, (hipStream_t)stream, *a, tpc, total);
    return VCR_LAUNCH_RC();
  }
  dim3 grid((a->N + PTS - 1) / PTS, a->B + a->B2);
  hipLaunchKernelGGL(pointwise12_kernel, grid, dim3(256), 0, (hipStream_t)stream, *a);
  return VCR_LAUNCH_RC();
}
```

vcr-net_amd/csrc/rigid_svd.hip:

```cpp
#include "common.h"

namespace {

__device__ __forceinline__ double wave_sum_f64(double v) {
#pragma unroll
  for (int o = 32; o >= 1; o >>= 1) v += __shfl_xor(v, o, 64);
  return v;
}
template <int NV>
__device__ __forceinline__ void block_sums(double (&v)[NV], double* red) {
  const int w = threadIdx.x >> 6;
#pragma unroll
  for (int e = 0; e < NV; ++e) v[e] = wave_sum_f64(v[e]);
  __syncthreads();
  if ((threadIdx.x & 63) == 0)
#pragma unroll
    for (int e = 0; e < NV; ++e) red[w * NV + e] = v[e];
  __syncthreads();
#pragma unroll
  for (int e = 0; e < NV; ++e) v[e] = ((red[e] + red[NV + e]) + red[2 * NV + e]) + red[3 * NV + e];
}
__device__ __forceinline__ double quad_xor(double v, int ctrl_is_1) {
  int lo = __double2loint(v), hi = __double2hiint(v);
  if (ctrl_is_1) { lo = __builtin_amdgcn_mov_dpp(lo, 0xB1, 0xF, 0xF, true); hi = __builtin_amdgcn_mov_dpp(hi, 0xB1, 0xF, 0xF, true); }
  else { lo = __builtin_amdgcn_mov_dpp(lo, 0x4E, 0xF, 0xF, true); hi = __builtin_amdgcn_mov_dpp(hi, 0x4E, 0xF, 0xF, true); }
  return __hiloint2double(hi, lo);
}
__device__ __forceinline__ double quad_sum(double v) {
  v += quad_xor(v, 1);
  v += quad_xor(v, 0);
  return v;
}
__device__ __forceinline__ double quad_get(double v, int lane_in_quad) {
  int lo = __double2loint(v), hi = __double2hiint(v);
  const int c = lane_in_quad == 0 ? 0x00 : lane_in_quad == 1 ? 0x55 : 0xAA;
  if (lane_in_quad == 0) { lo = __builtin_amdgcn_mov_dpp(lo, 0x00, 0xF, 0xF, true); hi = __builtin_amdgcn_mov_dpp(hi, 0x00, 0xF, 0xF, true); }
  else if (lane_in_quad == 1) { lo = __builtin_amdgcn_mov_dpp(lo, 0x55, 0xF, 0xF, true); hi = __builtin_amdgcn_mov_dpp(hi, 0x55, 0xF, 0xF, true); }
  else { lo = __builtin_amdgcn_mov_dpp(lo, 0xAA, 0xF, 0xF, true); hi = __builtin_amdgcn_mov_dpp(hi, 0xAA, 0xF, 0xF, true); }
  (void)c;
  return __hiloint2double(hi, lo);
}

__device__ __forceinline__ void jacobi_sweeps_quad(double (&a)[3], double (&v)[3]) {
  for (int sweep = 0; sweep < 40; ++sweep) {
    double off = 0.0;
#pragma unroll
    for (int pq = 0; pq < 3; ++pq) {
      const int p = (pq == 2) ? 1 : 0, q = (pq == 0) ? 1 : 2;
      const double al = quad_sum(a[p] * a[p]), be = quad_sum(a[q] * a[q]), ga = quad_sum(a[p] * a[q]);
      if (fabs(ga) <= 1e-30 + 1e-17 * sqrt(al * be)) continue;
      off = fmax(off, fabs(ga) / sqrt(al * be + 1e-300));
      const double zeta = (be - al) / (2.0 * ga);
      const double tt = (zeta >= 0 ? 1.0 : -1.0) / (fabs(zeta) + sqrt(1.0 + zeta * zeta));
      const double c = 1.0 / sqrt(1.0 + tt * tt), s = c * tt;
      const double ap = a[p], aq = a[q];
      a[p] = c * ap - s * aq; a[q] = s * ap + c * aq;
      const double vp = v[p], vq = v[q];
      v[p] = c * vp - s * vq; v[q] = s * vp + c * vq;
    }
    if (off < 1e-15) break;
  }
}

__device__ void svd3_finish(const double A[3][3], const double V[3][3], double R[9]) {
  double sig[3];
  int ord[3] = {0, 1, 2};
  for (int j = 0; j < 3; ++j) sig[j] = sqrt(A[0][j] * A[0][j] + A[1][j] * A[1][j] + A[2][j] * A[2][j]);
  for (int i = 0; i < 2; ++i)
    for (int j = 0; j < 2 - i; ++j)
      if (sig[ord[j]] < sig[ord[j + 1]]) { const int tmp = ord[j]; ord[j] = ord[j + 1]; ord[j + 1] = tmp; }
  double U[3][3], W[3][3];
  for (int j = 0; j < 3; ++j) {
    const int c = ord[j];
    const double inv = sig[c] > 0 ? 1.0 / sig[c] : 0.0;
    for (int i = 0; i < 3; ++i) { U[i][j] = A[i][c] * inv; W[i][j] = V[i][c]; }
  }
  const double s0 = sig[ord[0]];
  if (!(s0 > 1e-300)) {
    for (int i = 0; i < 3; ++i) for (int j = 0; j < 3; ++j) U[i][j] = W[i][j];
  } else {
    if (sig[ord[1]] <= 1e-12 * s0) {
      int e = 0;
      for (int i = 1; i < 3; ++i) if (fabs(U[i][0]) < fabs(U[e][0])) e = i;
      double v[3] = {0, 0, 0}, n2 = 0;
      v[e] = 1.0;
      const double d = U[e][0];
      for (int i = 0; i < 3; ++i) { v[i] -= d * U[i][0]; n2 += v[i] * v[i]; }
      const double inv = 1.0 / sqrt(n2);
      for (int i = 0; i < 3; ++i) U[i][1] = v[i] * inv;
    }
    if (sig[ord[2]] <= 1e-12 * s0) {
      U[0][2] = U[1][0] * U[2][1] - U[2][0] * U[1][1];
      U[1][2] = U[2][0] * U[0][1] - U[0][0] * U[2][1];
      U[2][2] = U[0][0] * U[1][1] - U[1][0] * U[0][1];
    }
  }
  auto build = [&]() {
    for (int i = 0; i < 3; ++i)
      for (int j = 0; j < 3; ++j) R[3 * i + j] = W[i][0] * U[j][0] + W[i][1] * U[j][1] + W[i][2] * U[j][2];
  };
  build();
  const double det = R[0] * (R[4] * R[8] - R[5] * R[7]) - R[1] * (R[3] * R[8] - R[5] * R[6]) +
                     R[2] * (R[3] * R[7] - R[4] * R[6]);
  if (det < 0) {
    for (int i = 0; i < 3; ++i) W[i][2] = -W[i][2];
    build();
  }
}

__global__ __launch_bounds__(256) void rigid_svd_kernel(vcr_rigid_svd_args p) {
  __shared__ double red[4 * 9];
  const int b = blockIdx.x, t = threadIdx.x;
  const float* S = p.src + (size_t)b * p.K * p.lds;
  const float* C = p.corr + (size_t)b * p.K * p.ldc;
  double mean[6] = {0, 0, 0, 0, 0, 0};
  for (int i = t; i < p.K; i += 256)
    for (int c = 0; c < 3; ++c) { mean[c] += S[(size_t)i * p.lds + c]; mean[3 + c] += C[(size_t)i * p.ldc + c]; }
  block_sums<6>(mean, red);
  float smf[3], cmf[3];
  for (int c = 0; c < 3; ++c) { smf[c] = (float)(mean[c] / p.K); cmf[c] = (float)(mean[3 + c] / p.K); }
  double H[9] = {0, 0, 0, 0, 0, 0, 0, 0, 0};
  for (int i = t; i < p.K; i += 256) {
    float sc[3], cc[3];
    for (int c = 0; c < 3; ++c) { sc[c] = S[(size_t)i * p.lds + c] - smf[c]; cc[c] = C[(size_t)i * p.ldc + c] - cmf[c]; }
    for (int r = 0; r < 3; ++r)
      for (int c = 0; c < 3; ++c) H[3 * r + c] += (double)sc[r] * (double)cc[c];
  }
  block_sums<9>(H, red);
  if (t >= 64) return;
  const int li = t & 3;
  double a[3], v[3];
#pragma unroll
  for (int j = 0; j < 3; ++j) {
    a[j] = li == 0 ? H[j] : li == 1 ? H[3 + j] : li == 2 ? H[6 + j] : 0.0;
    v[j] = li == j ? 1.0 : 0.0;
  }
  jacobi_sweeps_quad(a, v);
  double A[3][3], V[3][3];
#pragma unroll
  for (int j = 0; j < 3; ++j) {
    A[0][j] = quad_get(a[j], 0); A[1][j] = quad_get(a[j], 1); A[2][j] = quad_get(a[j], 2);
    V[0][j] = quad_get(v[j], 0); V[1][j] = quad_get(v[j], 1); V[2][j] = quad_get(v[j], 2);
  }
  if (t == 0) {
    double R[9];
    svd3_finish(A, V, R);
    bool finite = true;
    for (int e = 0; e < 9; ++e) finite = finite && __builtin_isfinite(H[e]);
    for (int c = 0; c < 6; ++c) finite = finite && __builtin_isfinite(mean[c]);
    if (!finite)
      for (int e = 0; e < 9; ++e) R[e] = __builtin_nan("");
    float* Ro = p.R + (size_t)b * 9;
    float* to = p.t + (size_t)b * 3;
    float Rf[9], tf[3];
    for (int e = 0; e < 9; ++e) { Rf[e] = (float)R[e]; Ro[e] = Rf[e]; }
    for (int r = 0; r < 3; ++r) {
      tf[r] = (float)(-(R[3 * r] * smf[0] + R[3 * r + 1] * smf[1] + R[3 * r + 2] * smf[2]) + cmf[r]);
      to[r] = tf[r];
    }
    if (p.R_ba) for (int r = 0; r < 3; ++r) for (int c = 0; c < 3; ++c) p.R_ba[(size_t)b * 9 + 3 * r + c] = Rf[3 * c + r];
    if (p.t_ba) for (int r = 0; r < 3; ++r)
      p.t_ba[(size_t)b * 3 + r] = -(Rf[r] * tf[0] + Rf[3 + r] * tf[1] + Rf[6 + r] * tf[2]);
    if (p.H) for (int e = 0; e < 9; ++e) p.H[(size_t)b * 9 + e] = (float)H[e];
  }
}

}

extern "C" int vcr_rigid_svd_f32(const vcr_rigid_svd_args* a, vcr_stream_t stream) {
  if (!a || !a->src || !a->corr || !a->R || !a->t) return VCR_EINVAL;
  if (a->B <= 0 || a->K < 3 || a->lds < 3 || a->ldc < 3) return VCR_EINVAL;
  hipLaunchKernelGGL(rigid_svd_kernel, dim3(a->B), dim3(256), 0, (hipStream_t)stream, *a);
  return VCR_LAUNCH_RC();
}
```

Baseline: 3226 pairs/s.

## Fuse rigid SVD into softcorr tail and fold zeroing/src4 copy into stem

The rigid SVD solve now runs in the last-arriving block of the softcorr pairscore kernel for each batch, using an atomic arrival counter and release/acquire fences. The separate zero-init kernel and the src4 device-to-device copy are folded into the pointwise stem kernel, which also zeroes the tie buffer and the arrival counters. This removes up to three launches and their serialization gaps. In exchange it adds atomics and a single-block tail solve. The fused path applies only when the head plan has a single split and cycle mode is off.

Measured after the change: 3231 pairs/s (median of 6 runs). About the same (+0.2%).

```diff
diff --git a/vcr-net_amd/csrc/forward.hip b/vcr-net_amd/csrc/forward.hip
--- a/vcr-net_amd/csrc/forward.hip
+++ b/vcr-net_amd/csrc/forward.hip
@@ -57,6 +57,7 @@
 struct Ws {
   float *xyz4, *feat64, *sq64, *pq1, *cat, *pq3, *emb;
   int32_t *idx1, *idx3, *ties;
+  int32_t* arrive;
   unsigned char* tie_work[2]; size_t tie_work_each;
   float* feat64t;
   float *feat_p, *xyz4_p, *cen64, *cen4, *sq_p, *c64_sq, *c64_rad, *c64_max, *c4_rad, *c4_max;
@@ -92,6 +93,10 @@
 extern "C" int vcr_knn_forms_(const vcr_knn_args* a, const vcr_knn_args* b, int* ordered, int* inline_a, int* inline_b);
 extern "C" int vcr_sdpa_forms_(const vcr_sdpa_args* a, int* nsplit, int* persistent);
 extern "C" long vcr_sdpa_split_floats_(size_t rows, int heads, int ldo, long nbatch, int nq, int cus);
+extern "C" int vcr_pointwise_stem_(const vcr_pointwise_args* a, int32_t* zero_a, long n_a, int32_t* zero_b, long n_b, float* src4,
+                                   long src4_rows, vcr_stream_t stream);
+extern "C" int vcr_softcorr_forms_(const vcr_softcorr_args* a, vcr_stream_t stream, int* nsplit);
+extern "C" int vcr_softcorr_solve_(const vcr_softcorr_args* a, const vcr_rigid_svd_args* s, int32_t* arrive, vcr_stream_t stream);
 
 Ws carve(void* base, const vcr_vcrnet_weights* W, int B, int N, int cus, int pass = 0) {
   const int k = W->k, E = W->E, F = W->F, heads = W->heads;
@@ -121,6 +126,7 @@
   pl.want(w.d2, M * E, DEC_CROSS_WO, END);
   pl.want(w.d3, M * E, DEC_FFN2, END);
   pl.want(w.embf, M * E, DEC_NORM, END);  pl.want(w.side4, M * 4, DEC_NORM, END);
+  pl.want(w.arrive, ((size_t)B + 3) & ~(size_t)3, STEM, END);
   pl.want(w.csplit, VCR_PAIRSCORE_MAX_SPLIT * (M / 2) * 8, HEAD, END);
   pl.want(w.corr_ba, (size_t)B * N * 4, HEAD2, END);
   w.asplit_floats = vcr_sdpa_split_floats_(2 * M, heads, E, 2L * B, N, cus);
@@ -189,9 +195,10 @@
   return w;
 }
 
-__global__ __launch_bounds__(256) void zero_i32_kernel(int32_t* p, long n) {
+__global__ __launch_bounds__(256) void zero_i32_kernel(int32_t* p, long n, int32_t* q, long m) {
   const long i = (long)blockIdx.x * 256 + threadIdx.x;
   if (i < n) p[i] = 0;
+  else if (i - n < m) q[i - n] = 0;
 }
 
 struct Runner {
@@ -459,8 +466,14 @@
   Runner R{(hipStream_t)stream, tr};
   R.shape_rows = half ? M2 : 0;
   R.plan_nbatch = half ? 2 * B : 0;
-  hipLaunchKernelGGL(zero_i32_kernel, dim3((unsigned)((M2 + 2 + 255) / 256)), dim3(256), 0, R.stream, w.ties, (long)(M2 + 2));
-  R.ok(VCR_LAUNCH_RC());
+  const long n_ties = (long)M2 + 2, n_arrive = B;
+  const bool stem_side = W->emb_kind == 0 && W->linear_mode == 0;
+  const bool src4_by_stem = stem_side && !(W->partial && W->head_mode == 0) && (((uintptr_t)io->src4) & 15) == 0;
+  if (!stem_side) {
+    hipLaunchKernelGGL(zero_i32_kernel, dim3((unsigned)((n_ties + n_arrive + 255) / 256)), dim3(256), 0, R.stream, w.ties, n_ties,
+                       w.arrive, n_arrive);
+    R.ok(VCR_LAUNCH_RC());
+  }
 #define SP(site) (W->linear_mode != 0 ? W->split.site : nullptr)
   R.sdpa_split = W->linear_mode == 2;
   R.sdpa_variant = W->sdpa_variant;
@@ -526,6 +539,7 @@
                          half ? 0 : B};
     if (pq_fused) { a.pq_w = W->dg1_wpq; a.pq_b = W->dg1_bpq; a.pq = w.pq1; a.ldpq = 256; }
     a.feat64t = w.feat64t;
+    if (stem_side) return vcr_pointwise_stem_(&a, w.ties, n_ties, w.arrive, n_arrive, src4_by_stem ? io->src4 : nullptr, M1, R.stream);
     return vcr_pointwise_f32(&a, R.stream);
   });
   const int32_t* rank_perm = nullptr;
@@ -638,24 +652,32 @@
     });
     head_emb = w.d3;
   }
+  auto soft_args = [&](size_t q0, size_t k0, float* corr) {
+    return vcr_softcorr_args{head_emb + q0 * E, E, head_emb + k0 * E, E, side + q0 * 4, side + k0 * 4,
+                             corr, B, N, N, E, W->head_mode == 1 ? 1 : 0, 1.0f / sqrtf((float)E), w.csplit,
+                             (long)VCR_PAIRSCORE_MAX_SPLIT * B * N * 8};
+  };
   auto soft_head = [&](const char* nm, size_t q0, size_t k0, float* corr) {
     R.run(nm, [&] {
-      vcr_softcorr_args a{head_emb + q0 * E, E, head_emb + k0 * E, E, side + q0 * 4, side + k0 * 4,
-                          corr, B, N, N, E, W->head_mode == 1 ? 1 : 0, 1.0f / sqrtf((float)E), w.csplit,
-                          (long)VCR_PAIRSCORE_MAX_SPLIT * B * N * 8};
+      const vcr_softcorr_args a = soft_args(q0, k0, corr);
       return vcr_softcorr_f32(&a, R.stream);
     });
   };
   if (hard_pairs) {
     R.partial_head(W, io, w, B, N);
   } else {
-    soft_head("softcorr:head", 0, (size_t)M1, io->corr4);
-    R.run("rigid_svd:ab", [&] {
-      const int c = vcr_copy_d2d(io->src4, w.xyz4, (size_t)M1 * 4 * sizeof(float), R.stream);
-      vcr_rigid_svd_args a{w.xyz4, 4, io->corr4, 4, B, N, io->R_ab, io->t_ab, io->R_ba, io->t_ba, nullptr};
-      const int s = vcr_rigid_svd_f32(&a, R.stream);
-      return c ? c : s;
-    });
+    const vcr_rigid_svd_args solve{w.xyz4, 4, io->corr4, 4, B, N, io->R_ab, io->t_ab, io->R_ba, io->t_ba, nullptr};
+    int head_runs = 0;
+    const vcr_softcorr_args ha = soft_args(0, (size_t)M1, io->corr4);
+    const bool solve_on_head = R.rc == 0 && !W->cycle && vcr_softcorr_forms_(&ha, R.stream, &head_runs) == VCR_OK && head_runs == 1;
+    if (solve_on_head) R.run("softcorr:head+svd", [&] { return vcr_softcorr_solve_(&ha, &solve, w.arrive, R.stream); });
+    else soft_head("softcorr:head", 0, (size_t)M1, io->corr4);
+    if (!src4_by_stem || !solve_on_head)
+      R.run(solve_on_head ? "select:src4.out" : "rigid_svd:ab", [&] {
+        const int c = src4_by_stem ? 0 : vcr_copy_d2d(io->src4, w.xyz4, (size_t)M1 * 4 * sizeof(float), R.stream);
+        const int s = solve_on_head ? 0 : vcr_rigid_svd_f32(&solve, R.stream);
+        return c ? c : s;
+      });
     if (W->cycle) {
       if (!io->R_ba || !io->t_ba) return VCR_EINVAL;
       if (W->head_mode == 2) {
diff --git a/vcr-net_amd/csrc/pairscore.hip b/vcr-net_amd/csrc/pairscore.hip
--- a/vcr-net_amd/csrc/pairscore.hip
+++ b/vcr-net_amd/csrc/pairscore.hip
@@ -1,6 +1,8 @@
-#include "common.h"
+#include "rigid_solve.h"
 
 namespace {
+
+struct PsSolve { int32_t* arrive; vcr_rigid_svd_args svd; };
 
 constexpr float LOG2E = 1.4426950408889634f;
 
@@ -10,7 +12,7 @@
 }
 
 template <int OP, int OT>
-__global__ __launch_bounds__(128 * OT * 2, (OT == 1 ? 2 : 1)) void pairscore_kernel(vcr_pairscore_args p, int nsplit) {
+__global__ __launch_bounds__(128 * OT * 2, (OT == 1 ? 2 : 1)) void pairscore_kernel(vcr_pairscore_args p, int nsplit, PsSolve tail) {
   extern __shared__ __attribute__((aligned(16))) unsigned char smem[];
   constexpr int NW = 4 * OT;
   constexpr int NO = 32 * OT;
@@ -52,7 +54,6 @@
   const float* sbase = p.str + (size_t)sb * p.n_str * p.ld_str;
   const float* sside = p.str_side4 ? p.str_side4 + (size_t)sb * p.n_str * 4 : nullptr;
   const float* sstat = (OP == 2) ? p.str_stat2 + (size_t)sb * p.str_stat_batch_stride : nullptr;
-
   f32x4 bufA[8], bufB[8];
   auto load_chunk = [&](int flat, f32x4* dst) {
     const int tile = t0 + w + NW * (flat / chunks), c = flat % chunks;
@@ -229,6 +230,26 @@
       st[orow * 2] = M; st[orow * 2 + 1] = L;
       if (p.argmax) p.argmax[orow] = Bi < p.n_str ? Bi : 0;
     }
+  }
+  if constexpr (OP == 0) {
+    if (!tail.arrive) return;
+    asm volatile("s_waitcnt vmcnt(0)" ::: "memory");
+    __syncthreads();
+    int* last = reinterpret_cast<int*>(mg) + 128;
+    if (t == 0) {
+      __builtin_amdgcn_fence(__ATOMIC_RELEASE, "agent");
+      asm volatile("s_waitcnt vmcnt(0)" ::: "memory");
+      const int seen = __hip_atomic_fetch_add(tail.arrive + b, 1, __ATOMIC_RELAXED, __HIP_MEMORY_SCOPE_AGENT);
+      const int mine = seen == (int)gridDim.x - 1;
+      if (mine) {
+        __builtin_amdgcn_fence(__ATOMIC_ACQUIRE, "agent");
+        asm volatile("s_waitcnt vmcnt(0)" ::: "memory");
+      }
+      *last = mine;
+    }
+    __syncthreads();
+    if (!*last) return;
+    rigid_solve_block(tail.svd, b, reinterpret_cast<double*>(mg));
   }
 }
 
@@ -354,15 +375,15 @@
   return VCR_OK;
 }
 
-}
-
-extern "C" int vcr_pairscore_f32(const vcr_pairscore_args* a, vcr_stream_t stream) {
+int pairscore_launch(const vcr_pairscore_args* a, vcr_stream_t stream, const PsSolve* tail) {
   vcr_stream_scope bound(stream);
   PairscorePlan p;
   int rc = pairscore_plan(a, &p);
   if (rc) return rc;
+  if (tail && (p.op != 0 || p.nsplit != 1)) return VCR_EINVAL;
+  const PsSolve ts = tail ? *tail : PsSolve{};
   hipStream_t s = (hipStream_t)stream;
-#define VCR_PS(OP, OT) rc = vcr_launch<pairscore_kernel<OP, OT>>(p.grid, p.block, p.lds, s, *a, p.nsplit)
+#define VCR_PS(OP, OT) rc = vcr_launch<pairscore_kernel<OP, OT>>(p.grid, p.block, p.lds, s, *a, p.nsplit, ts)
   if (p.ot == 2) { if (p.op == 0) VCR_PS(0, 2); else if (p.op == 1) VCR_PS(1, 2); else VCR_PS(2, 2); }
   else           { if (p.op == 0) VCR_PS(0, 1); else if (p.op == 1) VCR_PS(1, 1); else VCR_PS(2, 1); }
 #undef VCR_PS
@@ -372,6 +393,20 @@
   return VCR_LAUNCH_RC();
 }
 
+vcr_pairscore_args softcorr_pairscore_args(const vcr_softcorr_args* a) {
+  vcr_pairscore_args p{};
+  p.own = a->q; p.ld_own = a->ldq; p.str = a->k; p.ld_str = a->ldk;
+  p.own_side4 = a->qside4; p.str_side4 = a->kside4;
+  p.nbatch = a->nbatch; p.n_own = a->nq; p.n_str = a->nk; p.E = a->E;
+  p.score = a->mode; p.scale = a->scale; p.str_batch_shift = 0; p.op = 0; p.corr4 = a->corr4;
+  p.split_work = a->split_work; p.split_work_floats = a->split_work_floats;
+  return p;
+}
+
+}
+
+extern "C" int vcr_pairscore_f32(const vcr_pairscore_args* a, vcr_stream_t stream) { return pairscore_launch(a, stream, nullptr); }
+
 extern "C" int vcr_scoremass_f32(const vcr_scoremass_args* a, vcr_stream_t stream) {
   if (!a || !a->score || !a->row_stat2 || !a->col_stat2 || !a->col_mass || !a->row_mass) return VCR_EINVAL;
   if (a->nbatch <= 0 || a->n_rows <= 0 || a->n_cols <= 0 || a->ld < a->n_cols) return VCR_EINVAL;
@@ -384,11 +419,24 @@
 extern "C" int vcr_softcorr_f32(const vcr_softcorr_args* a, vcr_stream_t stream) {
   if (!a || !a->qside4 || !a->kside4 || !a->corr4) return VCR_EINVAL;
   if (a->mode != 0 && a->mode != 1) return VCR_EINVAL;
-  vcr_pairscore_args p{};
-  p.own = a->q; p.ld_own = a->ldq; p.str = a->k; p.ld_str = a->ldk;
-  p.own_side4 = a->qside4; p.str_side4 = a->kside4;
-  p.nbatch = a->nbatch; p.n_own = a->nq; p.n_str = a->nk; p.E = a->E;
-  p.score = a->mode; p.scale = a->scale; p.str_batch_shift = 0; p.op = 0; p.corr4 = a->corr4;
-  p.split_work = a->split_work; p.split_work_floats = a->split_work_floats;
-  return vcr_pairscore_f32(&p, stream);
-}
+  const vcr_pairscore_args p = softcorr_pairscore_args(a);
+  return pairscore_launch(&p, stream, nullptr);
+}
+
+extern "C" int vcr_softcorr_forms_(const vcr_softcorr_args* a, vcr_stream_t stream, int* nsplit) {
+  if (!a || !a->qside4 || !a->kside4 || !a->corr4 || (a->mode != 0 && a->mode != 1)) return VCR_EINVAL;
+  vcr_stream_scope bound(stream);
+  const vcr_pairscore_args p = softcorr_pairscore_args(a);
+  PairscorePlan pl;
+  const int rc = pairscore_plan(&p, &pl);
+  if (rc == VCR_OK && nsplit) *nsplit = pl.nsplit;
+  return rc;
+}
+extern "C" int vcr_softcorr_solve_(const vcr_softcorr_args* a, const vcr_rigid_svd_args* s, int32_t* arrive, vcr_stream_t stream) {
+  if (!a || !a->qside4 || !a->kside4 || !a->corr4 || (a->mode != 0 && a->mode != 1)) return VCR_EINVAL;
+  if (!s || !arrive || !s->src || !s->R || !s->t || s->corr != a->corr4 || s->ldc != 4 || s->lds < 3) return VCR_EINVAL;
+  if (s->B != a->nbatch || s->K != a->nq || s->K < 3) return VCR_EINVAL;
+  const vcr_pairscore_args p = softcorr_pairscore_args(a);
+  const PsSolve tail{arrive, *s};
+  return pairscore_launch(&p, stream, &tail);
+}
diff --git a/vcr-net_amd/csrc/pointwise.hip b/vcr-net_amd/csrc/pointwise.hip
--- a/vcr-net_amd/csrc/pointwise.hip
+++ b/vcr-net_amd/csrc/pointwise.hip
@@ -97,9 +97,10 @@
   }
 }
 
+struct PwSide { int32_t* zero_a; long n_a; int32_t* zero_b; long n_b; float* rows4_copy; long copy_rows; };
 constexpr int TP = 68;
 constexpr int PQW = 8;
-__global__ __launch_bounds__(64 * PQW, 1) void pointwise12_pq_kernel(vcr_pointwise_args a, int tiles_per_cloud, int total_tiles) {
+__global__ __launch_bounds__(64 * PQW, 1) void pointwise12_pq_kernel(vcr_pointwise_args a, int tiles_per_cloud, int total_tiles, PwSide side) {
   extern __shared__ __attribute__((aligned(16))) float pw_smem[];
   float* wfrag = pw_smem;
   float* w1s = wfrag + 16 * 4 * 64 * 4;
@@ -107,6 +108,8 @@
   float* tiles = pqb + 256;
   const int t = threadIdx.x, lane = t & 63, wave = t >> 6;
   const int q4 = lane >> 4, l15 = lane & 15;
+  for (long i = (long)blockIdx.x * (64 * PQW) + t; i < side.n_a; i += (long)gridDim.x * (64 * PQW)) side.zero_a[i] = 0;
+  for (long i = (long)blockIdx.x * (64 * PQW) + t; i < side.n_b; i += (long)gridDim.x * (64 * PQW)) side.zero_b[i] = 0;
   f32x4 w2c[4][4];
 #pragma unroll
   for (int j = 0; j < 4; ++j)
@@ -218,7 +221,9 @@
         }
         if (g == 0) {
           a.sq64[row] = ss;
-          st4(a.xyz4 + row * 4, f32x4{x, y, z, (x * x + y * y) + z * z});
+          const f32x4 r4{x, y, z, (x * x + y * y) + z * z};
+          st4(a.xyz4 + row * 4, r4);
+          if ((long)row < side.copy_rows) st4(side.rows4_copy + row * 4, r4);
         }
       }
     };
@@ -309,7 +314,7 @@
   return VCR_LAUNCH_RC();
 }
 
-extern "C" int vcr_pointwise_f32(const vcr_pointwise_args* a, vcr_stream_t stream) {
+static int pointwise_launch(const vcr_pointwise_args* a, vcr_stream_t stream, const PwSide* side) {
   vcr_stream_scope bound(stream);
   if (!a || !a->x_cf || !a->w1 || !a->b1 || !a->w2 || !a->b2 || !a->xyz4 || !a->feat64 || !a->sq64) return VCR_EINVAL;
   if (((uintptr_t)a->w2 | (uintptr_t)a->pq_w) & 15) return VCR_EINVAL;
@@ -320,10 +325,22 @@
     const int cus = vcr_cu_count(), blocks = (total + PQW - 1) / PQW < cus ? (total + PQW - 1) / PQW : cus;
     const size_t lds = (size_t)(16 * 4 * 64 * 4 + 64 * 4 + 256 + PQW * 16 * TP) * sizeof(float);
     VCR_DYN_LDS(pointwise12_pq_kernel, lds);
-    hipLaunchKernelGGL(pointwise12_pq_kernel, dim3(blocks), dim3(64 * PQW), lds, (hipStream_t)stream, *a, tpc, total);
+    hipLaunchKernelGGL(pointwise12_pq_kernel, dim3(blocks), dim3(64 * PQW), lds, (hipStream_t)stream, *a, tpc, total,
+                       side ? *side : PwSide{});
     return VCR_LAUNCH_RC();
   }
+  if (side) return VCR_EINVAL;
   dim3 grid((a->N + PTS - 1) / PTS, a->B + a->B2);
   hipLaunchKernelGGL(pointwise12_kernel, grid, dim3(256), 0, (hipStream_t)stream, *a);
   return VCR_LAUNCH_RC();
 }
+
+extern "C" int vcr_pointwise_f32(const vcr_pointwise_args* a, vcr_stream_t stream) { return pointwise_launch(a, stream, nullptr); }
+
+extern "C" int vcr_pointwise_stem_(const vcr_pointwise_args* a, int32_t* zero_a, long n_a, int32_t* zero_b, long n_b, float* src4,
+                                   long src4_rows, vcr_stream_t stream) {
+  if (!a || !a->pq || n_a < 0 || n_b < 0 || (n_a && !zero_a) || (n_b && !zero_b) || src4_rows < 0) return VCR_EINVAL;
+  if (src4 && (((uintptr_t)src4 & 15) || src4_rows > (long)(a->B + a->B2) * a->N)) return VCR_EINVAL;
+  const PwSide side{zero_a, n_a, zero_b, n_b, src4, src4 ? src4_rows : 0};
+  return pointwise_launch(a, stream, &side);
+}
diff --git a/vcr-net_amd/csrc/rigid_solve.h b/vcr-net_amd/csrc/rigid_solve.h
--- /dev/null
+++ b/vcr-net_amd/csrc/rigid_solve.h
@@ -0,0 +1,214 @@
+#pragma once
+#include "common.h"
+
+namespace {
+
+__device__ __forceinline__ double wave_sum_f64(double v) {
+#pragma unroll
+  for (int o = 32; o >= 1; o >>= 1) v += __shfl_xor(v, o, 64);
+  return v;
+}
+template <int NV>
+__device__ __forceinline__ void block_sums(double (&v)[NV], double* red) {
+  const int w = threadIdx.x >> 6;
+#pragma unroll
+  for (int e = 0; e < NV; ++e) v[e] = wave_sum_f64(v[e]);
+  __syncthreads();
+  if ((threadIdx.x & 63) == 0 && w < 4)
+#pragma unroll
+    for (int e = 0; e < NV; ++e) red[w * NV + e] = v[e];
+  __syncthreads();
+#pragma unroll
+  for (int e = 0; e < NV; ++e) v[e] = ((red[e] + red[NV + e]) + red[2 * NV + e]) + red[3 * NV + e];
+}
+__device__ __forceinline__ double quad_xor(double v, int ctrl_is_1) {
+  int lo = __double2loint(v), hi = __double2hiint(v);
+  if (ctrl_is_1) { lo = __builtin_amdgcn_mov_dpp(lo, 0xB1, 0xF, 0xF, true); hi = __builtin_amdgcn_mov_dpp(hi, 0xB1, 0xF, 0xF, true); }
+  else { lo = __builtin_amdgcn_mov_dpp(lo, 0x4E, 0xF, 0xF, true); hi = __builtin_amdgcn_mov_dpp(hi, 0x4E, 0xF, 0xF, true); }
+  return __hiloint2double(hi, lo);
+}
+__device__ __forceinline__ double quad_sum(double v) {
+  v += quad_xor(v, 1);
+  v += quad_xor(v, 0);
+  return v;
+}
+__device__ __forceinline__ double quad_get(double v, int lane_in_quad) {
+  int lo = __double2loint(v), hi = __double2hiint(v);
+  const int c = lane_in_quad == 0 ? 0x00 : lane_in_quad == 1 ? 0x55 : 0xAA;
+  if (lane_in_quad == 0) { lo = __builtin_amdgcn_mov_dpp(lo, 0x00, 0xF, 0xF, true); hi = __builtin_amdgcn_mov_dpp(hi, 0x00, 0xF, 0xF, true); }
+  else if (lane_in_quad == 1) { lo = __builtin_amdgcn_mov_dpp(lo, 0x55, 0xF, 0xF, true); hi = __builtin_amdgcn_mov_dpp(hi, 0x55, 0xF, 0xF, true); }
+  else { lo = __builtin_amdgcn_mov_dpp(lo, 0xAA, 0xF, 0xF, true); hi = __builtin_amdgcn_mov_dpp(hi, 0xAA, 0xF, 0xF, true); }
+  (void)c;
+  return __hiloint2double(hi, lo);
+}
+
+__device__ __forceinline__ void jacobi_sweeps_quad(double (&a)[3], double (&v)[3]) {
+  for (int sweep = 0; sweep < 40; ++sweep) {
+    double off = 0.0;
+#pragma unroll
+    for (int pq = 0; pq < 3; ++pq) {
+      const int p = (pq == 2) ? 1 : 0, q = (pq == 0) ? 1 : 2;
+      const double al = quad_sum(a[p] * a[p]), be = quad_sum(a[q] * a[q]), ga = quad_sum(a[p] * a[q]);
+      if (fabs(ga) <= 1e-30 + 1e-17 * sqrt(al * be)) continue;
+      off = fmax(off, fabs(ga) / sqrt(al * be + 1e-300));
+      const double zeta = (be - al) / (2.0 * ga);
+      const double tt = (zeta >= 0 ? 1.0 : -1.0) / (fabs(zeta) + sqrt(1.0 + zeta * zeta));
+      const double c = 1.0 / sqrt(1.0 + tt * tt), s = c * tt;
+      const double ap = a[p], aq = a[q];
+      a[p] = c * ap - s * aq; a[q] = s * ap + c * aq;
+      const double vp = v[p], vq = v[q];
+      v[p] = c * vp - s * vq; v[q] = s * vp + c * vq;
+    }
+    if (off < 1e-15) break;
+  }
+}
+
+__device__ __forceinline__ double pick3(double x0, double x1, double x2, int c) { return c == 0 ? x0 : c == 1 ? x1 : x2; }
+__device__ __forceinline__ void svd3_finish(const double A[3][3], const double V[3][3], double R[9]) {
+  double sig[3];
+#pragma unroll
+  for (int j = 0; j < 3; ++j) sig[j] = sqrt(A[0][j] * A[0][j] + A[1][j] * A[1][j] + A[2][j] * A[2][j]);
+  int ord[3] = {0, 1, 2};
+  auto sg = [&](int c) { return pick3(sig[0], sig[1], sig[2], c); };
+  if (sg(ord[0]) < sg(ord[1])) { const int tmp = ord[0]; ord[0] = ord[1]; ord[1] = tmp; }
+  if (sg(ord[1]) < sg(ord[2])) { const int tmp = ord[1]; ord[1] = ord[2]; ord[2] = tmp; }
+  if (sg(ord[0]) < sg(ord[1])) { const int tmp = ord[0]; ord[0] = ord[1]; ord[1] = tmp; }
+  double U[3][3], W[3][3];
+#pragma unroll
+  for (int j = 0; j < 3; ++j) {
+    const int c = ord[j];
+    const double sc = sg(c);
+    const double inv = sc > 0 ? 1.0 / sc : 0.0;
+#pragma unroll
+    for (int i = 0; i < 3; ++i) { U[i][j] = pick3(A[i][0], A[i][1], A[i][2], c) * inv; W[i][j] = pick3(V[i][0], V[i][1], V[i][2], c); }
+  }
+  const double s0 = sg(ord[0]);
+  if (!(s0 > 1e-300)) {
+#pragma unroll
+    for (int i = 0; i < 3; ++i)
+#pragma unroll
+      for (int j = 0; j < 3; ++j) U[i][j] = W[i][j];
+  } else {
+    if (sg(ord[1]) <= 1e-12 * s0) {
+      int e = 0;
+#pragma unroll
+      for (int i = 1; i < 3; ++i) if (fabs(U[i][0]) < fabs(pick3(U[0][0], U[1][0], U[2][0], e))) e = i;
+      double v[3], n2 = 0;
+      const double d = pick3(U[0][0], U[1][0], U[2][0], e);
+#pragma unroll
+      for (int i = 0; i < 3; ++i) { v[i] = (i == e ? 1.0 : 0.0) - d * U[i][0]; n2 += v[i] * v[i]; }
+      const double inv = 1.0 / sqrt(n2);
+#pragma unroll
+      for (int i = 0; i < 3; ++i) U[i][1] = v[i] * inv;
+    }
+    if (sg(ord[2]) <= 1e-12 * s0) {
+      U[0][2] = U[1][0] * U[2][1] - U[2][0] * U[1][1];
+      U[1][2] = U[2][0] * U[0][1] - U[0][0] * U[2][1];
+      U[2][2] = U[0][0] * U[1][1] - U[1][0] * U[0][1];
+    }
+  }
+  auto build = [&]() {
+#pragma unroll
+    for (int i = 0; i < 3; ++i)
+#pragma unroll
+      for (int j = 0; j < 3; ++j) R[3 * i + j] = W[i][0] * U[j][0] + W[i][1] * U[j][1] + W[i][2] * U[j][2];
+  };
+  build();
+  const double det = R[0] * (R[4] * R[8] - R[5] * R[7]) - R[1] * (R[3] * R[8] - R[5] * R[6]) +
+                     R[2] * (R[3] * R[7] - R[4] * R[6]);
+  if (det < 0) {
+#pragma unroll
+    for (int i = 0; i < 3; ++i) W[i][2] = -W[i][2];
+    build();
+  }
+}
+
+__device__ __forceinline__ void rigid_solve_block(const vcr_rigid_svd_args& p, int b, double* red) {
+  const int t = threadIdx.x;
+  const int first = t < 256 ? t : p.K;
+  const float* S = p.src + (size_t)b * p.K * p.lds;
+  const float* C = p.corr + (size_t)b * p.K * p.ldc;
+  const bool cached = p.lds == 4 && p.ldc == 4 && p.K <= 1024 && ((((uintptr_t)p.src) | ((uintptr_t)p.corr)) & 15) == 0;
+  f32x4 sr[4], cr[4];
+  if (cached) {
+#pragma unroll
+    for (int j = 0; j < 4; ++j) {
+      const int i = first + 256 * j;
+      sr[j] = cr[j] = f32x4{0.f, 0.f, 0.f, 0.f};
+      if (i < p.K) { sr[j] = ld4(S + (size_t)i * 4); cr[j] = ld4(C + (size_t)i * 4); }
+    }
+  }
+  double mean[6] = {0, 0, 0, 0, 0, 0};
+  if (cached) {
+#pragma unroll
+    for (int j = 0; j < 4; ++j)
+      if (first + 256 * j < p.K)
+        for (int c = 0; c < 3; ++c) { mean[c] += sr[j][c]; mean[3 + c] += cr[j][c]; }
+  } else {
+    for (int i = first; i < p.K; i += 256)
+      for (int c = 0; c < 3; ++c) { mean[c] += S[(size_t)i * p.lds + c]; mean[3 + c] += C[(size_t)i * p.ldc + c]; }
+  }
+  block_sums<6>(mean, red);
+  float smf[3], cmf[3];
+  for (int c = 0; c < 3; ++c) { smf[c] = (float)(mean[c] / p.K); cmf[c] = (float)(mean[3 + c] / p.K); }
+  double H[9] = {0, 0, 0, 0, 0, 0, 0, 0, 0};
+  auto add_pair = [&](const float (&s3)[3], const float (&c3)[3]) {
+    float sc[3], cc[3];
+    for (int c = 0; c < 3; ++c) { sc[c] = s3[c] - smf[c]; cc[c] = c3[c] - cmf[c]; }
+    for (int r = 0; r < 3; ++r)
+      for (int c = 0; c < 3; ++c) H[3 * r + c] += (double)sc[r] * (double)cc[c];
+  };
+  if (cached) {
+#pragma unroll
+    for (int j = 0; j < 4; ++j)
+      if (first + 256 * j < p.K) {
+        const float s3[3] = {sr[j][0], sr[j][1], sr[j][2]}, c3[3] = {cr[j][0], cr[j][1], cr[j][2]};
+        add_pair(s3, c3);
+      }
+  } else {
+    for (int i = first; i < p.K; i += 256) {
+      const float s3[3] = {S[(size_t)i * p.lds], S[(size_t)i * p.lds + 1], S[(size_t)i * p.lds + 2]};
+      const float c3[3] = {C[(size_t)i * p.ldc], C[(size_t)i * p.ldc + 1], C[(size_t)i * p.ldc + 2]};
+      add_pair(s3, c3);
+    }
+  }
+  block_sums<9>(H, red);
+  if (t >= 64) return;
+  const int li = t & 3;
+  double a[3], v[3];
+#pragma unroll
+  for (int j = 0; j < 3; ++j) {
+    a[j] = li == 0 ? H[j] : li == 1 ? H[3 + j] : li == 2 ? H[6 + j] : 0.0;
+    v[j] = li == j ? 1.0 : 0.0;
+  }
+  jacobi_sweeps_quad(a, v);
+  double A[3][3], V[3][3];
+#pragma unroll
+  for (int j = 0; j < 3; ++j) {
+    A[0][j] = quad_get(a[j], 0); A[1][j] = quad_get(a[j], 1); A[2][j] = quad_get(a[j], 2);
+    V[0][j] = quad_get(v[j], 0); V[1][j] = quad_get(v[j], 1); V[2][j] = quad_get(v[j], 2);
+  }
+  if (t == 0) {
+    double R[9];
+    svd3_finish(A, V, R);
+    bool finite = true;
+    for (int e = 0; e < 9; ++e) finite = finite && __builtin_isfinite(H[e]);
+    for (int c = 0; c < 6; ++c) finite = finite && __builtin_isfinite(mean[c]);
+    if (!finite)
+      for (int e = 0; e < 9; ++e) R[e] = __builtin_nan("");
+    float* Ro = p.R + (size_t)b * 9;
+    float* to = p.t + (size_t)b * 3;
+    float Rf[9], tf[3];
+    for (int e = 0; e < 9; ++e) { Rf[e] = (float)R[e]; Ro[e] = Rf[e]; }
+    for (int r = 0; r < 3; ++r) {
+      tf[r] = (float)(-(R[3 * r] * smf[0] + R[3 * r + 1] * smf[1] + R[3 * r + 2] * smf[2]) + cmf[r]);
+      to[r] = tf[r];
+    }
+    if (p.R_ba) for (int r = 0; r < 3; ++r) for (int c = 0; c < 3; ++c) p.R_ba[(size_t)b * 9 + 3 * r + c] = Rf[3 * c + r];
+    if (p.t_ba) for (int r = 0; r < 3; ++r)
+      p.t_ba[(size_t)b * 3 + r] = -(Rf[r] * tf[0] + Rf[3 + r] * tf[1] + Rf[6 + r] * tf[2]);
+    if (p.H) for (int e = 0; e < 9; ++e) p.H[(size_t)b * 9 + e] = (float)H[e];
+  }
+}
+
+}
diff --git a/vcr-net_amd/csrc/rigid_svd.hip b/vcr-net_amd/csrc/rigid_svd.hip
--- a/vcr-net_amd/csrc/rigid_svd.hip
+++ b/vcr-net_amd/csrc/rigid_svd.hip
@@ -1,168 +1,10 @@
-#include "common.h"
+#include "rigid_solve.h"
 
 namespace {
 
-__device__ __forceinline__ double wave_sum_f64(double v) {
-#pragma unroll
-  for (int o = 32; o >= 1; o >>= 1) v += __shfl_xor(v, o, 64);
-  return v;
-}
-template <int NV>
-__device__ __forceinline__ void block_sums(double (&v)[NV], double* red) {
-  const int w = threadIdx.x >> 6;
-#pragma unroll
-  for (int e = 0; e < NV; ++e) v[e] = wave_sum_f64(v[e]);
-  __syncthreads();
-  if ((threadIdx.x & 63) == 0)
-#pragma unroll
-    for (int e = 0; e < NV; ++e) red[w * NV + e] = v[e];
-  __syncthreads();
-#pragma unroll
-  for (int e = 0; e < NV; ++e) v[e] = ((red[e] + red[NV + e]) + red[2 * NV + e]) + red[3 * NV + e];
-}
-__device__ __forceinline__ double quad_xor(double v, int ctrl_is_1) {
-  int lo = __double2loint(v), hi = __double2hiint(v);
-  if (ctrl_is_1) { lo = __builtin_amdgcn_mov_dpp(lo, 0xB1, 0xF, 0xF, true); hi = __builtin_amdgcn_mov_dpp(hi, 0xB1, 0xF, 0xF, true); }
-  else { lo = __builtin_amdgcn_mov_dpp(lo, 0x4E, 0xF, 0xF, true); hi = __builtin_amdgcn_mov_dpp(hi, 0x4E, 0xF, 0xF, true); }
-  return __hiloint2double(hi, lo);
-}
-__device__ __forceinline__ double quad_sum(double v) {
-  v += quad_xor(v, 1);
-  v += quad_xor(v, 0);
-  return v;
-}
-__device__ __forceinline__ double quad_get(double v, int lane_in_quad) {
-  int lo = __double2loint(v), hi = __double2hiint(v);
-  const int c = lane_in_quad == 0 ? 0x00 : lane_in_quad == 1 ? 0x55 : 0xAA;
-  if (lane_in_quad == 0) { lo = __builtin_amdgcn_mov_dpp(lo, 0x00, 0xF, 0xF, true); hi = __builtin_amdgcn_mov_dpp(hi, 0x00, 0xF, 0xF, true); }
-  else if (lane_in_quad == 1) { lo = __builtin_amdgcn_mov_dpp(lo, 0x55, 0xF, 0xF, true); hi = __builtin_amdgcn_mov_dpp(hi, 0x55, 0xF, 0xF, true); }
-  else { lo = __builtin_amdgcn_mov_dpp(lo, 0xAA, 0xF, 0xF, true); hi = __builtin_amdgcn_mov_dpp(hi, 0xAA, 0xF, 0xF, true); }
-  (void)c;
-  return __hiloint2double(hi, lo);
-}
-
-__device__ __forceinline__ void jacobi_sweeps_quad(double (&a)[3], double (&v)[3]) {
-  for (int sweep = 0; sweep < 40; ++sweep) {
-    double off = 0.0;
-#pragma unroll
-    for (int pq = 0; pq < 3; ++pq) {
-      const int p = (pq == 2) ? 1 : 0, q = (pq == 0) ? 1 : 2;
-      const double al = quad_sum(a[p] * a[p]), be = quad_sum(a[q] * a[q]), ga = quad_sum(a[p] * a[q]);
-      if (fabs(ga) <= 1e-30 + 1e-17 * sqrt(al * be)) continue;
-      off = fmax(off, fabs(ga) / sqrt(al * be + 1e-300));
-      const double zeta = (be - al) / (2.0 * ga);
-      const double tt = (zeta >= 0 ? 1.0 : -1.0) / (fabs(zeta) + sqrt(1.0 + zeta * zeta));
-      const double c = 1.0 / sqrt(1.0 + tt * tt), s = c * tt;
-      const double ap = a[p], aq = a[q];
-      a[p] = c * ap - s * aq; a[q] = s * ap + c * aq;
-      const double vp = v[p], vq = v[q];
-      v[p] = c * vp - s * vq; v[q] = s * vp + c * vq;
-    }
-    if (off < 1e-15) break;
-  }
-}
-
-__device__ void svd3_finish(const double A[3][3], const double V[3][3], double R[9]) {
-  double sig[3];
-  int ord[3] = {0, 1, 2};
-  for (int j = 0; j < 3; ++j) sig[j] = sqrt(A[0][j] * A[0][j] + A[1][j] * A[1][j] + A[2][j] * A[2][j]);
-  for (int i = 0; i < 2; ++i)
-    for (int j = 0; j < 2 - i; ++j)
-      if (sig[ord[j]] < sig[ord[j + 1]]) { const int tmp = ord[j]; ord[j] = ord[j + 1]; ord[j + 1] = tmp; }
-  double U[3][3], W[3][3];
-  for (int j = 0; j < 3; ++j) {
-    const int c = ord[j];
-    const double inv = sig[c] > 0 ? 1.0 / sig[c] : 0.0;
-    for (int i = 0; i < 3; ++i) { U[i][j] = A[i][c] * inv; W[i][j] = V[i][c]; }
-  }
-  const double s0 = sig[ord[0]];
-  if (!(s0 > 1e-300)) {
-    for (int i = 0; i < 3; ++i) for (int j = 0; j < 3; ++j) U[i][j] = W[i][j];
-  } else {
-    if (sig[ord[1]] <= 1e-12 * s0) {
-      int e = 0;
-      for (int i = 1; i < 3; ++i) if (fabs(U[i][0]) < fabs(U[e][0])) e = i;
-      double v[3] = {0, 0, 0}, n2 = 0;
-      v[e] = 1.0;
-      const double d = U[e][0];
-      for (int i = 0; i < 3; ++i) { v[i] -= d * U[i][0]; n2 += v[i] * v[i]; }
-      const double inv = 1.0 / sqrt(n2);
-      for (int i = 0; i < 3; ++i) U[i][1] = v[i] * inv;
-    }
-    if (sig[ord[2]] <= 1e-12 * s0) {
-      U[0][2] = U[1][0] * U[2][1] - U[2][0] * U[1][1];
-      U[1][2] = U[2][0] * U[0][1] - U[0][0] * U[2][1];
-      U[2][2] = U[0][0] * U[1][1] - U[1][0] * U[0][1];
-    }
-  }
-  auto build = [&]() {
-    for (int i = 0; i < 3; ++i)
-      for (int j = 0; j < 3; ++j) R[3 * i + j] = W[i][0] * U[j][0] + W[i][1] * U[j][1] + W[i][2] * U[j][2];
-  };
-  build();
-  const double det = R[0] * (R[4] * R[8] - R[5] * R[7]) - R[1] * (R[3] * R[8] - R[5] * R[6]) +
-                     R[2] * (R[3] * R[7] - R[4] * R[6]);
-  if (det < 0) {
-    for (int i = 0; i < 3; ++i) W[i][2] = -W[i][2];
-    build();
-  }
-}
-
 __global__ __launch_bounds__(256) void rigid_svd_kernel(vcr_rigid_svd_args p) {
   __shared__ double red[4 * 9];
-  const int b = blockIdx.x, t = threadIdx.x;
-  const float* S = p.src + (size_t)b * p.K * p.lds;
-  const float* C = p.corr + (size_t)b * p.K * p.ldc;
-  double mean[6] = {0, 0, 0, 0, 0, 0};
-  for (int i = t; i < p.K; i += 256)
-    for (int c = 0; c < 3; ++c) { mean[c] += S[(size_t)i * p.lds + c]; mean[3 + c] += C[(size_t)i * p.ldc + c]; }
-  block_sums<6>(mean, red);
-  float smf[3], cmf[3];
-  for (int c = 0; c < 3; ++c) { smf[c] = (float)(mean[c] / p.K); cmf[c] = (float)(mean[3 + c] / p.K); }
-  double H[9] = {0, 0, 0, 0, 0, 0, 0, 0, 0};
-  for (int i = t; i < p.K; i += 256) {
-    float sc[3], cc[3];
-    for (int c = 0; c < 3; ++c) { sc[c] = S[(size_t)i * p.lds + c] - smf[c]; cc[c] = C[(size_t)i * p.ldc + c] - cmf[c]; }
-    for (int r = 0; r < 3; ++r)
-      for (int c = 0; c < 3; ++c) H[3 * r + c] += (double)sc[r] * (double)cc[c];
-  }
-  block_sums<9>(H, red);
-  if (t >= 64) return;
-  const int li = t & 3;
-  double a[3], v[3];
-#pragma unroll
-  for (int j = 0; j < 3; ++j) {
-    a[j] = li == 0 ? H[j] : li == 1 ? H[3 + j] : li == 2 ? H[6 + j] : 0.0;
-    v[j] = li == j ? 1.0 : 0.0;
-  }
-  jacobi_sweeps_quad(a, v);
-  double A[3][3], V[3][3];
-#pragma unroll
-  for (int j = 0; j < 3; ++j) {
-    A[0][j] = quad_get(a[j], 0); A[1][j] = quad_get(a[j], 1); A[2][j] = quad_get(a[j], 2);
-    V[0][j] = quad_get(v[j], 0); V[1][j] = quad_get(v[j], 1); V[2][j] = quad_get(v[j], 2);
-  }
-  if (t == 0) {
-    double R[9];
-    svd3_finish(A, V, R);
-    bool finite = true;
-    for (int e = 0; e < 9; ++e) finite = finite && __builtin_isfinite(H[e]);
-    for (int c = 0; c < 6; ++c) finite = finite && __builtin_isfinite(mean[c]);
-    if (!finite)
-      for (int e = 0; e < 9; ++e) R[e] = __builtin_nan("");
-    float* Ro = p.R + (size_t)b * 9;
-    float* to = p.t + (size_t)b * 3;
-    float Rf[9], tf[3];
-    for (int e = 0; e < 9; ++e) { Rf[e] = (float)R[e]; Ro[e] = Rf[e]; }
-    for (int r = 0; r < 3; ++r) {
-      tf[r] = (float)(-(R[3 * r] * smf[0] + R[3 * r + 1] * smf[1] + R[3 * r + 2] * smf[2]) + cmf[r]);
-      to[r] = tf[r];
-    }
-    if (p.R_ba) for (int r = 0; r < 3; ++r) for (int c = 0; c < 3; ++c) p.R_ba[(size_t)b * 9 + 3 * r + c] = Rf[3 * c + r];
-    if (p.t_ba) for (int r = 0; r < 3; ++r)
-      p.t_ba[(size_t)b * 3 + r] = -(Rf[r] * tf[0] + Rf[3 + r] * tf[1] + Rf[6 + r] * tf[2]);
-    if (p.H) for (int e = 0; e < 9; ++e) p.H[(size_t)b * 9 + e] = (float)H[e];
-  }
+  rigid_solve_block(p, blockIdx.x, red);
 }
 
 }
```
